# marbl/Mash

Hardware: AMD Instinct MI355X
Metric: pairwise Mash distances/sec (s=1000) (higher is better)
Workload: dtype u64; 1 GPU; mash triangle all-vs-all, 100000 clustered synthetic sketches, k=21 s=1000, 4999950000 pairs/step, per-table job (index build + discover + fill + merge each step), row-block sharded x1; parallelism=rowblock1, rccl_ranks=0

## Files before the change

### mash_amd/csrc/compare_dense.hip

```cpp
#ifdef MG_HIP_EMU
#include "hipemu.h"
#else
#include <hip/hip_runtime.h>
#define MG_DYN_SHARED(T, name)                                   \
    extern __shared__ __align__(16) unsigned char name##_raw[]; \
    T *name = reinterpret_cast<T *>(name##_raw)
#endif
#include <stdint.h>

#include <cstdlib>

#ifndef MG_HIP_EMU
#include <rocprim/device/device_radix_sort.hpp>
#include <rocprim/device/device_select.hpp>
#include <rocprim/iterator/counting_iterator.hpp>
#endif

#include "compare_internal.h"

namespace mg {

#ifndef MG_HIP_EMU
__global__ __launch_bounds__(256) void dn_neighbor_kernel(const uint64_t *hashes, uint64_t stride, const uint32_t *cnt, uint32_t n,
                                                          uint8_t *link)
{
    const uint32_t row = blockIdx.x * 4u + (threadIdx.x >> 6), lane = threadIdx.x & 63u;
    if (row >= n) return;
    uint32_t hit = 0;
    uint32_t ci = 0, cj = 0;
    if (row > 0) {
        ci = cnt[row];
        cj = cnt[row - 1];
        const uint32_t take = ci < 64u ? ci : 64u, span = cj < 256u ? cj : 256u;
        if (lane < take && span > 0) {
            const uint64_t v = hashes[(uint64_t)row * stride + lane];
            const uint64_t *q = hashes + (uint64_t)(row - 1) * stride;
            uint32_t lo = 0, hi = span;
            while (lo < hi) {
                const uint32_t mid = (lo + hi) >> 1;
                if (q[mid] < v) lo = mid + 1; else hi = mid;
            }
            hit = (lo < span && q[lo] == v) ? 1u : 0u;
        }
    }
    const uint32_t hits = (uint32_t)__popcll(__ballot(hit != 0));
    const uint32_t take = ci < 64u ? ci : 64u;
    if (lane == 0) link[row] = (row > 0 && take >= 16u && cj >= 16u && 2u * hits >= take) ? 1 : 0;
}

hipError_t launch_dense_neighbors(const uint64_t *hashes, uint64_t stride, const uint32_t *cnt, uint32_t n, uint8_t *link,
                                  hipStream_t stream)
{
    if (n == 0) return hipSuccess;
    hipLaunchKernelGGL(dn_neighbor_kernel, dim3((n + 3u) / 4u), dim3(256), 0, stream, hashes, stride, cnt, n, link);
    return hipGetLastError();
}

constexpr uint32_t DN_SUBLISTS = 1024;

__global__ __launch_bounds__(256) void dn_leaders_kernel(const uint32_t *sorted_rows, const uint32_t *gs_of, const uint32_t *gend,
                                                         const uint32_t *grp_of, const DenseGroup *groups, uint32_t E,
                                                         unsigned long long *key, uint32_t *val, uint32_t cap_sub, uint32_t *cnt)
{
    const uint32_t pos = blockIdx.x * 256u + threadIdx.x;
    bool lead = false;
    uint32_t g = 0xFFFFFFFFu, gs = 0;
    if (pos < E) {
        g = grp_of[sorted_rows[pos]];
        if (g != 0xFFFFFFFFu) {
            const uint32_t g0 = groups[g].g0, g1 = groups[g].g1;
            gs = gs_of[pos];
            const bool first = pos == gs || sorted_rows[pos - 1] < g0;
            const bool more = pos + 1u < gend[gs] && sorted_rows[pos + 1] < g1;
            lead = first && more;
        }
    }
    const uint64_t bal = __ballot(lead);
    if (bal == 0) return;
    const uint32_t lane = threadIdx.x & 63u, sub = blockIdx.x & (DN_SUBLISTS - 1u);
    uint32_t base = 0;
    if (lane == (uint32_t)__builtin_ctzll(bal)) base = atomicAdd(&cnt[sub], (uint32_t)__popcll(bal));
    base = (uint32_t)__builtin_amdgcn_readlane((int)base, __builtin_ctzll(bal));
    if (lead) {
        const uint32_t k = base + (uint32_t)__popcll(bal & ((1ull << lane) - 1ull));
        if (k < cap_sub) {
            const uint64_t slot = (uint64_t)sub * cap_sub + k;
            key[slot] = ((unsigned long long)g << 32) | gs;
            val[slot] = pos;
        }
    }
}

__global__ __launch_bounds__(DN_SUBLISTS) void dn_sublists_scan_kernel(const uint32_t *cnt, uint32_t cap_sub, uint32_t *off, uint32_t *total)
{
    __shared__ uint32_t s_w[DN_SUBLISTS / 64];
    const uint32_t t = threadIdx.x, lane = t & 63u, wid = t >> 6;
    const uint32_t want = cnt[t], c = want < cap_sub ? want : cap_sub;
    uint32_t incl = c;
#pragma unroll
    for (int d = 1; d < 64; d <<= 1) {
        const uint32_t x = __shfl_up(incl, d);
        if (lane >= (uint32_t)d) incl += x;
    }
    if (lane == 63u) s_w[wid] = incl;
    __syncthreads();
    uint32_t base = 0;
    for (uint32_t k = 0; k < wid; k++) base += s_w[k];
    off[t] = base + incl - c;
    if (t == DN_SUBLISTS - 1u) total[0] = base + incl;
    atomicMax(&total[1], want);
}

__global__ __launch_bounds__(256) void dn_sublists_copy_kernel(const unsigned long long *key, const uint32_t *val, const uint32_t *cnt,
                                                               const uint32_t *off, uint32_t cap_sub, unsigned long long *key_out,
                                                               uint32_t *val_out)
{
    const uint32_t sub = blockIdx.x;
    const uint32_t c = cnt[sub] < cap_sub ? cnt[sub] : cap_sub, o = off[sub];
    for (uint32_t k = threadIdx.x; k < c; k += 256u) {
        key_out[o + k] = key[(uint64_t)sub * cap_sub + k];
        val_out[o + k] = val[(uint64_t)sub * cap_sub + k];
    }
}

__global__ __launch_bounds__(256) void dn_universe_split_kernel(const unsigned long long *key_sorted, uint32_t m, uint32_t *ulist,
                                                                uint32_t *ustart, uint32_t *uend)
{
    const uint32_t i = blockIdx.x * 256u + threadIdx.x;
    if (i >= m) return;
    const unsigned long long k = key_sorted[i];
    const uint32_t g = (uint32_t)(k >> 32);
    ulist[i] = (uint32_t)k;
    if (i == 0 || (uint32_t)(key_sorted[i - 1] >> 32) != g) ustart[g] = i;
    if (i + 1u == m || (uint32_t)(key_sorted[i + 1] >> 32) != g) uend[g] = i + 1u;
}

size_t dense_universe_temp_bytes(uint32_t cap)
{
    size_t b = 0;
    rocprim::radix_sort_pairs(nullptr, b, (const unsigned long long *)nullptr, (unsigned long long *)nullptr, (const uint32_t *)nullptr,
                              (uint32_t *)nullptr, (size_t)cap, 0u, 64u, (hipStream_t) nullptr);
    return b;
}

uint32_t dense_sublists() { return DN_SUBLISTS; }

hipError_t dense_find_leaders(const uint32_t *sorted_rows, const uint32_t *gs_of, const uint32_t *gend, const uint32_t *grp_of,
                              const DenseGroup *groups, uint32_t E, unsigned long long *key, uint32_t *val, uint32_t cap_sub,
                              unsigned long long *key_out, uint32_t *val_out, uint32_t *cnt, uint32_t *off, uint32_t *total,
                              hipStream_t stream)
{
    if (E == 0) return hipSuccess;
    hipError_t e = hipMemsetAsync(cnt, 0, DN_SUBLISTS * 4, stream);
    if (e == hipSuccess) e = hipMemsetAsync(total, 0, 8, stream);
    if (e != hipSuccess) return e;
    hipLaunchKernelGGL(dn_leaders_kernel, dim3((E + 255u) / 256u), dim3(256), 0, stream, sorted_rows, gs_of, gend, grp_of, groups, E, key, val, cap_sub,
                       cnt);
    e = hipGetLastError();
    if (e != hipSuccess) return e;
    return dense_join_leaders(key, val, cap_sub, key_out, val_out, cnt, off, total, stream);
}

hipError_t dense_join_leaders(const unsigned long long *key, const uint32_t *val, uint32_t cap_sub, unsigned long long *key_out, uint32_t *val_out,
                              const uint32_t *cnt, uint32_t *off, uint32_t *total, hipStream_t stream)
{
    hipLaunchKernelGGL(dn_sublists_scan_kernel, dim3(1), dim3(DN_SUBLISTS), 0, stream, cnt, cap_sub, off, total);
    hipLaunchKernelGGL(dn_sublists_copy_kernel, dim3(DN_SUBLISTS), dim3(256), 0, stream, key, val, cnt, (const uint32_t *)off, cap_sub, key_out, val_out);
    return hipGetLastError();
}

hipError_t dense_sort_universes(const unsigned long long *key, const uint32_t *val, uint32_t m, void *temp, size_t temp_bytes,
                                unsigned long long *key_sorted, uint32_t *ulist, uint32_t *upos, uint32_t *ustart, uint32_t *uend,
                                uint32_t group_bits, hipStream_t stream)
{
    if (m == 0) return hipSuccess;
    hipError_t e = rocprim::radix_sort_pairs(temp, temp_bytes, key, key_sorted, val, upos, (size_t)m, 0u, 32u + group_bits, stream);
    if (e != hipSuccess) return e;
    hipLaunchKernelGGL(dn_universe_split_kernel, dim3((m + 255u) / 256u), dim3(256), 0, stream, (const unsigned long long *)key_sorted, m, ulist,
                       ustart, uend);
    return hipGetLastError();
}

#endif

constexpr uint32_t DN_CX_MASK = 0x7FFFu, DN_CX_FLAG = 0x8000u;

struct DnEncodeOpts {
    uint32_t ul_in_lds;
    uint32_t *row_any;
#ifdef __HIPCC__
    __host__ __device__
#endif
    DnEncodeOpts(uint32_t ul, uint32_t *flags = nullptr) : ul_in_lds(ul), row_any(flags) {}
};

template <uint32_t DN_EK>
__global__ __launch_bounds__(256) void dn_encode_kernel(const uint32_t *off, const uint32_t *code_img, uint32_t *pos_img, uint32_t rs,
                                                        const uint32_t *grp_of, const DenseGroup *groups, const uint32_t *ulist,
                                                        const uint32_t *upos, unsigned long long *gdata, uint32_t wstride, uint16_t *ext,
                                                        uint32_t xs, uint32_t n, DnEncodeOpts opt)
{
    MG_DYN_SHARED(uint32_t, lds);
    const uint32_t bid = blockIdx.x;
    const uint32_t row = (bid & ~63u) | ((bid & 7u) << 3) | ((bid >> 3) & 7u);
    const uint32_t tid = threadIdx.x, lane = tid & 63u, wid = tid >> 6;
    if (row >= n) return;
    const uint32_t g = grp_of[row];
    if (g == 0xFFFFFFFFu) return;
    const DenseGroup G = groups[g];
    const uint32_t W = G.W, u = G.u;
    uint32_t *mask32 = lds, *hist = lds + 2u * W, *gap8 = hist + W + 1u, *ovf = gap8 + 16u * W, *pl32 = ovf + W, *scr = pl32 + 8u * W;
    uint32_t *ull = lds + 28u * wstride + 9u;
    for (uint32_t i = tid; i < 28u * W + 1u; i += 256u) lds[i] = 0;
    const uint32_t *ulg = ulist + G.ustart, *up = upos + G.ustart;
    if (opt.ul_in_lds)
        for (uint32_t i = tid; i < u; i += 256u) ull[i] = ulg[i];
    const uint32_t *ul = opt.ul_in_lds ? ull : ulg;
    if (tid == 0) scr[4] = 0;
    __syncthreads();
    const uint32_t cnt = off[row + 1] - off[row];
    uint16_t *xrow = ext + (uint64_t)(G.xrow0 + (row - G.g0)) * xs;
    uint32_t nx = 0;
    bool any = false;
    if constexpr (DN_EK == 1) {
        for (uint32_t base = 0; base < cnt; base += 256u) {
            const uint32_t p = base + tid;
            uint32_t idx = 0;
            bool extra = false;
            if (p < cnt) {
                const uint64_t img = (uint64_t)row * rs + p;
                const uint32_t code = code_img[img], gs = code >> 1;
                uint32_t lo = 0, hi = u;
                while (lo < hi) {
                    const uint32_t mid = (lo + hi) >> 1;
                    if (ul[mid] < gs) lo = mid + 1; else hi = mid;
                }
                idx = lo;
                if (lo < u && ul[lo] == gs) {
                    atomicOr(&mask32[idx >> 5], 1u << (idx & 31u));
                    const uint32_t end = up[idx];
                    pos_img[img] = end;
                    any |= end != gs;
                } else {
                    extra = true;
                    if (opt.row_any && (code & 1u)) any |= pos_img[img] != gs;
                }
            }
            const uint64_t bal = __ballot(extra);
            const uint32_t before = (uint32_t)__popcll(bal & ((1ull << lane) - 1ull));
            if (lane == 0) scr[wid] = (uint32_t)__popcll(bal);
            __syncthreads();
            uint32_t woff = 0;
            for (uint32_t k = 0; k < wid; k++) woff += scr[k];
            const uint32_t total = scr[0] + scr[1] + scr[2] + scr[3];
            if (extra) {
                xrow[nx + woff + before] = (uint16_t)idx;
                atomicAdd(&hist[idx >> 6], 1u);
                atomicAdd(&gap8[idx >> 2], 1u << (8u * (idx & 3u)));
            }
            nx += total;
            __syncthreads();
        }
    } else {
        for (uint32_t base = 0; base < cnt; base += 256u * DN_EK) {
            const uint32_t p0 = base + tid * DN_EK;
            const uint32_t nv = p0 < cnt ? (cnt - p0 < DN_EK ? cnt - p0 : DN_EK) : 0u;
            uint32_t xidx[DN_EK];
            uint32_t nxt = 0;
            if (nv) {
                const uint64_t img0 = (uint64_t)row * rs + p0;
                const uint4 c0 = *reinterpret_cast<const uint4 *>(code_img + img0), c1 = *reinterpret_cast<const uint4 *>(code_img + img0 + 4u);
                const uint32_t code[DN_EK] = {c0.x, c0.y, c0.z, c0.w, c1.x, c1.y, c1.z, c1.w};
                uint4 *pp = reinterpret_cast<uint4 *>(pos_img + img0);
                const uint4 q0 = pp[0], q1 = pp[1];
                uint32_t pv[DN_EK] = {q0.x, q0.y, q0.z, q0.w, q1.x, q1.y, q1.z, q1.w};
                uint32_t pos = 0;
                {
                    const uint32_t gs0 = code[0] >> 1;
                    uint32_t lo = 0, hi = u;
                    while (lo < hi) {
                        const uint32_t mid = (lo + hi) >> 1;
                        if (ul[mid] < gs0) lo = mid + 1; else hi = mid;
                    }
                    pos = lo;
                }
    #pragma unroll
                for (uint32_t e = 0; e < DN_EK; e++) {
                    if (e < nv) {
                        const uint32_t gs = code[e] >> 1;
                        {
                            uint32_t lo = pos, hi = pos, step = 1;
                            while (hi < u && ul[hi] < gs) {
                                lo = hi + 1u;
                                hi += step;
                                step <<= 1;
                            }
                            hi = hi < u ? hi : u;
                            while (lo < hi) {
                                const uint32_t mid = (lo + hi) >> 1;
                                if (ul[mid] < gs) lo = mid + 1u; else hi = mid;
                            }
                            pos = lo;
                        }
                        if (pos < u && ul[pos] == gs) {
                            atomicOr(&mask32[pos >> 5], 1u << (pos & 31u));
                            pv[e] = up[pos];
                        } else {
    #pragma unroll
                            for (uint32_t j = 0; j < DN_EK; j++)
                                if (j == nxt) xidx[j] = pos;
                            nxt++;
                        }
                        any |= pv[e] != gs;
                    }
                }
                pp[0] = make_uint4(pv[0], pv[1], pv[2], pv[3]);
                pp[1] = make_uint4(pv[4], pv[5], pv[6], pv[7]);
            }
            uint32_t incl = nxt;
    #pragma unroll
            for (uint32_t d = 1; d < 64u; d <<= 1) {
                const uint32_t y = __shfl_up(incl, d);
                if (lane >= d) incl += y;
            }
            if (lane == 63u) scr[wid] = incl;
            __syncthreads();
            uint32_t woff = 0;
            for (uint32_t k = 0; k < wid; k++) woff += scr[k];
            const uint32_t total = scr[0] + scr[1] + scr[2] + scr[3];
            const uint32_t at0 = nx + woff + incl - nxt;
    #pragma unroll
            for (uint32_t j = 0; j < DN_EK; j++) {
                if (j < nxt) {
                    const uint32_t idx = xidx[j];
                    xrow[at0 + j] = (uint16_t)idx;
                    atomicAdd(&hist[idx >> 6], 1u);
                    atomicAdd(&gap8[idx >> 2], 1u << (8u * (idx & 3u)));
                }
            }
            nx += total;
            __syncthreads();
        }
    }
    if (__ballot(any) != 0 && lane == 0) atomicOr(&scr[4], 1u);
    __syncthreads();
    if (opt.row_any && tid == 0) opt.row_any[row] = scr[4];
    const uint32_t jb = (row - G.g0) >> 7, bl = (row - G.g0) & 127u;
    const uint64_t bw = dense_block_words(W);
    unsigned long long *blk = gdata + G.data_off + (uint64_t)jb * bw;
    uint16_t *cxp = reinterpret_cast<uint16_t *>(blk + 128ull * W), *totp = cxp + (W + 1u) * 128u;
    unsigned long long *xpl = blk + dense_block_planes(W);
    for (uint32_t i = tid; i < 16u * W; i += 256u) {
        const uint32_t four = gap8[i], w = i >> 4, q = i & 15u;
        uint32_t bits[4] = {0u, 0u, 0u, 0u}, over = 0;
#pragma unroll
        for (uint32_t e = 0; e < 4u; e++) {
            const uint32_t c = (four >> (8u * e)) & 255u;
            over |= c >= 16u ? 1u : 0u;
#pragma unroll
            for (uint32_t j = 0; j < 4u; j++) bits[j] |= ((c >> j) & 1u) << ((4u * q + e) & 31u);
        }
        if (over || (q == 0 && hist[w] >= 256u)) ovf[w] = 1u;
#pragma unroll
        for (uint32_t j = 0; j < 4u; j++)
            if (bits[j]) atomicOr(&pl32[2u * (4u * w + j) + (q >> 3)], bits[j]);
    }
    __syncthreads();
    for (uint32_t i = tid; i < 4u * W; i += 256u) xpl[i * 128u + bl] = (unsigned long long)pl32[2u * i] | ((unsigned long long)pl32[2u * i + 1u] << 32);
    if (tid == 0) {
        uint32_t run = 0, all = 0;
        for (uint32_t w = 0; w <= W; w++) {
            cxp[w * 128u + bl] = (uint16_t)(run | ((w > 0 && ovf[w - 1u]) ? DN_CX_FLAG : 0u));
            totp[w * 128u + bl] = (uint16_t)all;
            if (w < W) {
                run += hist[w];
                all += hist[w] + (uint32_t)__popc(mask32[2u * w]) + (uint32_t)__popc(mask32[2u * w + 1u]);
            }
        }
    }
    for (uint32_t w = tid; w < W; w += 256u)
        blk[w * 128u + bl] = (unsigned long long)mask32[2u * w] | ((unsigned long long)mask32[2u * w + 1u] << 32);
}

hipError_t launch_dense_encode(const uint32_t *off, const uint32_t *code_img, uint32_t *pos_img, uint32_t rs, const uint32_t *grp_of,
                               const DenseGroup *groups, const uint32_t *ulist, const uint32_t *upos, unsigned long long *gdata,
                               uint16_t *ext, uint32_t xs, uint32_t n, uint32_t wmax, hipStream_t stream, int ul_mode, uint32_t *row_any)
{
    if (n == 0) return hipSuccess;
    const size_t fixed = ((size_t)28 * wmax + 9) * 4, with_ul = fixed + (size_t)wmax * 64 * 4;
    const bool ul_in_lds = ul_mode == 0 ? false : ul_mode == 1 ? with_ul <= 150 * 1024 : with_ul <= 40 * 1024;
    const size_t smem = ul_in_lds ? with_ul : fixed;
    auto go = [&](auto kern) -> hipError_t {
        hipError_t e = hipFuncSetAttribute(reinterpret_cast<const void *>(kern), hipFuncAttributeMaxDynamicSharedMemorySize, (int)smem);
        if (e != hipSuccess) return e;
        hipLaunchKernelGGL(kern, dim3((n + 63u) & ~63u), dim3(256), smem, stream, off, code_img, pos_img, rs, grp_of, groups, ulist, upos, gdata, wmax, ext, xs,
                           n, DnEncodeOpts(ul_in_lds ? 1u : 0u, row_any));
        return hipGetLastError();
    };
    return rs >= 4096u ? go(dn_encode_kernel<8>) : go(dn_encode_kernel<1>);
}



__device__ __forceinline__ uint32_t dn_count_add(uint32_t x, uint32_t acc)
{
#ifdef MG_HIP_EMU
    return (uint32_t)__popc(x) + acc;
#else
    uint32_t d;
    asm("v_bcnt_u32_b32 %0, %1, %2" : "=v"(d) : "v"(x), "v"(acc));
    return d;
#endif
}

__device__ __forceinline__ uint32_t dn_low_bits(uint32_t x, uint32_t y)
{
#ifdef MG_HIP_EMU
    return x & ((1u << y) - 1u);
#else
    return __builtin_amdgcn_ubfe(x, 0u, y);
#endif
}

template <uint32_t NP>
__device__ __forceinline__ uint32_t dn_descend(uint32_t base, uint32_t s, uint32_t u1, uint32_t A0, uint32_t B0, uint32_t A1, uint32_t B1,
                                               uint32_t A2, uint32_t B2, uint32_t A3, uint32_t B3)
{
    uint32_t pos = 0;
#pragma unroll
    for (uint32_t bit = 16u; bit != 0u; bit >>= 1) {
        const uint32_t y = pos + bit;
        uint32_t c = dn_count_add(dn_low_bits(B0, y), dn_count_add(dn_low_bits(A0, y), dn_count_add(dn_low_bits(u1, y), base)));
        if (NP >= 1u) c += 2u * dn_count_add(dn_low_bits(B1, y), (uint32_t)__popc(dn_low_bits(A1, y)));
        if (NP >= 3u)
            c += 4u * dn_count_add(dn_low_bits(B2, y), (uint32_t)__popc(dn_low_bits(A2, y))) +
                 8u * dn_count_add(dn_low_bits(B3, y), (uint32_t)__popc(dn_low_bits(A3, y)));
        pos = c < s ? y : pos;
    }
    return pos;
}

__device__ __forceinline__ uint32_t dn_resolve(unsigned long long un, unsigned long long mab, uint32_t fprev, uint32_t s, uint32_t w, bool lists,
                                               const unsigned long long *xpa, const unsigned long long *xpb, const uint16_t *xa,
                                               const uint16_t *xb, uint32_t ca0, uint32_t na, uint32_t cb0, uint32_t nb)
{
    if (__ballot(lists) == 0) {
        const unsigned long long a0 = xpa[512u * w], a1 = xpa[512u * w + 128u], a2 = xpa[512u * w + 256u], a3 = xpa[512u * w + 384u];
        const unsigned long long b0 = xpb[512u * w], b1 = xpb[512u * w + 128u], b2 = xpb[512u * w + 256u], b3 = xpb[512u * w + 384u];
        const bool p1 = __ballot((a1 | b1) != 0ull) != 0, p23 = __ballot((a2 | a3 | b2 | b3) != 0ull) != 0;
        const uint32_t ulo = (uint32_t)un, uhi = (uint32_t)(un >> 32);
        uint32_t c31 = dn_count_add((uint32_t)b0, dn_count_add((uint32_t)a0, dn_count_add(ulo & 0x7FFFFFFFu, fprev)));
        if (p1 || p23) c31 += 2u * dn_count_add((uint32_t)b1, (uint32_t)__popc((uint32_t)a1));
        if (p23)
            c31 += 4u * dn_count_add((uint32_t)b2, (uint32_t)__popc((uint32_t)a2)) + 8u * dn_count_add((uint32_t)b3, (uint32_t)__popc((uint32_t)a3));
        const bool upper = c31 < s;
        const uint32_t base = upper ? c31 + (ulo >> 31) : fprev;
        const uint32_t u1 = (upper ? uhi : ulo) << 1;
        const uint32_t A0 = upper ? (uint32_t)(a0 >> 32) : (uint32_t)a0, B0 = upper ? (uint32_t)(b0 >> 32) : (uint32_t)b0;
        uint32_t pos;
        if (!p1 && !p23) {
            pos = dn_descend<0>(base, s, u1, A0, B0, 0, 0, 0, 0, 0, 0);
        } else {
            const uint32_t A1 = upper ? (uint32_t)(a1 >> 32) : (uint32_t)a1, B1 = upper ? (uint32_t)(b1 >> 32) : (uint32_t)b1;
            if (!p23) {
                pos = dn_descend<1>(base, s, u1, A0, B0, A1, B1, 0, 0, 0, 0);
            } else {
                const uint32_t A2 = upper ? (uint32_t)(a2 >> 32) : (uint32_t)a2, B2 = upper ? (uint32_t)(b2 >> 32) : (uint32_t)b2;
                const uint32_t A3 = upper ? (uint32_t)(a3 >> 32) : (uint32_t)a3, B3 = upper ? (uint32_t)(b3 >> 32) : (uint32_t)b3;
                pos = dn_descend<3>(base, s, u1, A0, B0, A1, B1, A2, B2, A3, B3);
            }
        }
        const uint32_t mlo = (uint32_t)mab, mhi = (uint32_t)(mab >> 32);
        return upper ? dn_count_add(dn_low_bits(mhi, pos), (uint32_t)__popc(mlo)) : (uint32_t)__popc(dn_low_bits(mlo, pos));
    }
    uint32_t lo = 0, hi = 63;
    const uint32_t wbase = w << 6;
    while (lo < hi) {
        const uint32_t mid = (lo + hi) >> 1;
        uint32_t c = fprev + (uint32_t)__popcll(un & ((1ull << mid) - 1ull));
        for (uint32_t k = 0; k < na; k++) c += ((uint32_t)xa[ca0 + k] - wbase <= mid) ? 1u : 0u;
        for (uint32_t k = 0; k < nb; k++) c += ((uint32_t)xb[cb0 + k] - wbase <= mid) ? 1u : 0u;
        if (c >= s) hi = mid; else lo = mid + 1u;
    }
    return (uint32_t)__popcll(mab & ((1ull << lo) - 1ull));
}

template <uint32_t DN_ROWS, uint32_t DN_IL>
__global__ __launch_bounds__(128) void dn_pairs_kernel(const DenseTile *tiles, const DenseGroup *groups, const unsigned long long *gdata,
                                                       uint32_t use_lists,
                                                       const uint16_t *ext, uint32_t xs, uint32_t s, uint32_t row_begin, uint32_t row_end,
                                                       uint64_t out_base, const uint32_t *inv, uint2 *out, DenseList list)
{
    MG_DYN_SHARED(unsigned long long, dl);
    const DenseTile T = tiles[blockIdx.x];
    const DenseGroup G = groups[T.group];
    const uint32_t W = G.W, tid = threadIdx.x;
    const uint64_t bw = dense_block_words(W);
    const unsigned long long *Bm = gdata + G.data_off + (uint64_t)T.cblk * bw;
    const uint16_t *Bcx = reinterpret_cast<const uint16_t *>(Bm + 128ull * W);
    const uint16_t *Btot = Bcx + (W + 1u) * 128u;
    unsigned long long *Am = dl;
    uint16_t *Acx = reinterpret_cast<uint16_t *>(Am + (uint64_t)DN_ROWS * W);
    uint16_t *Atot = Acx + (W + 1u) * DN_ROWS;
    const uint32_t ra = T.row0 - G.g0;
    const unsigned long long *asrc = gdata + G.data_off + (uint64_t)(ra >> 7) * bw;
    const uint32_t la0 = ra & 127u;
    for (uint32_t i = tid; i < W * DN_ROWS; i += 128u) Am[i] = asrc[(i / DN_ROWS) * 128u + la0 + (i % DN_ROWS)];
    {
        const uint16_t *acs = reinterpret_cast<const uint16_t *>(asrc + 128ull * W);
        for (uint32_t i = tid; i < 2u * (W + 1u) * DN_ROWS; i += 128u) Acx[i] = acs[(i / DN_ROWS) * 128u + la0 + (i % DN_ROWS)];
    }
    __syncthreads();
    constexpr uint32_t DN_NB = DN_ROWS / DN_IL;
    uint16_t *Amax = Atot + (W + 1u) * DN_ROWS;
    for (uint32_t i = tid; i < DN_NB * (W + 1u); i += 128u) {
        const uint32_t bt = i / (W + 1u), w = i - bt * (W + 1u);
        uint32_t m = 0;
        for (uint32_t k = 0; k < DN_IL; k++)
            if (T.row0 + bt * DN_IL + k < G.g1) {
                const uint32_t v = Atot[w * DN_ROWS + bt * DN_IL + k];
                m = v > m ? v : m;
            }
        Amax[i] = (uint16_t)m;
    }
    __syncthreads();
    const uint32_t b = G.g0 + T.cblk * 128u + tid;
    const uint32_t lb = b < G.g1 ? tid : G.g1 - 1u - (G.g0 + T.cblk * 128u);
    const uint16_t *xb = ext + (uint64_t)(G.xrow0 + (b < G.g1 ? b - G.g0 : 0u)) * xs;
    const unsigned long long *xpb = Bm + dense_block_planes(W) + lb;
    const uint32_t colrow = inv ? inv[G.g0 + T.cblk * 128u + lb] : G.g0 + T.cblk * 128u + lb;
    const uint64_t tri_col = (colrow ? (uint64_t)colrow * (colrow - 1u) / 2u : 0ull) - out_base;
    for (uint32_t ai = 0; ai < DN_ROWS; ai += DN_IL) {
        if (T.row0 + ai >= G.g1 || T.row0 + ai >= row_end) break;
        const uint16_t *amax = Amax + (ai / DN_IL) * (W + 1u);
        uint32_t common[DN_IL], nle[DN_IL];
#pragma unroll
        for (uint32_t k = 0; k < DN_IL; k++) common[k] = nle[k] = 0;
        unsigned long long mb_next = Bm[lb];
        uint32_t tb_next = Btot[128u + lb];
        uint32_t wi = 0;
        for (; wi < W; wi++) {
            if (__ballot((uint32_t)amax[wi + 1u] + tb_next > s) != 0) break;
            const unsigned long long mb = mb_next;
            if (wi + 1u < W) {
                mb_next = Bm[(wi + 1u) * 128u + lb];
                tb_next = Btot[(wi + 2u) * 128u + lb];
            }
            const uint32_t mlo = (uint32_t)mb, mhi = (uint32_t)(mb >> 32);
#pragma unroll
            for (uint32_t k = 0; k < DN_IL; k++) {
                const unsigned long long am = Am[wi * DN_ROWS + ai + k];
                common[k] = dn_count_add((uint32_t)am & mlo, dn_count_add((uint32_t)(am >> 32) & mhi, common[k]));
            }
        }
        const uint32_t nfast = wi;
        for (; wi < W; wi++) {
            const unsigned long long mb = mb_next;
            const int32_t tbs = (int32_t)tb_next - (int32_t)s;
            if (wi + 1u < W) {
                mb_next = Bm[(wi + 1u) * 128u + lb];
                tb_next = Btot[(wi + 2u) * 128u + lb];
            }
            const uint32_t mlo = (uint32_t)mb, mhi = (uint32_t)(mb >> 32);
            bool any = false;
#pragma unroll
            for (uint32_t k = 0; k < DN_IL; k++) {
                const unsigned long long am = Am[wi * DN_ROWS + ai + k];
                const uint32_t cnew = dn_count_add((uint32_t)am & mlo, dn_count_add((uint32_t)(am >> 32) & mhi, common[k]));
                const bool before = (int32_t)Atot[(wi + 1u) * DN_ROWS + ai + k] + tbs <= (int32_t)cnew;
                common[k] = before ? cnew : common[k];
                nle[k] += before ? 1u : 0u;
                any = any || before;
            }
            if (__ballot(any) == 0) break;
        }
#pragma unroll
        for (uint32_t k = 0; k < DN_IL; k++) {
            const uint32_t a = T.row0 + ai + k;
            const bool present = a < G.g1 && a < row_end && a >= row_begin && G.g0 + T.cblk * 128u < a;
            if (!present) continue;
            const bool valid = b < a;
            uint32_t denom = s;
            const uint32_t w = nfast + nle[k];
            const bool need = valid && w < W;
            if (__ballot(need) != 0) {
                const uint32_t wc = need ? w : 0u;
                const unsigned long long ma = Am[wc * DN_ROWS + ai + k], mb = Bm[wc * 128u + lb];
                const uint32_t ca0 = Acx[wc * DN_ROWS + ai + k] & DN_CX_MASK, ca1r = Acx[(wc + 1u) * DN_ROWS + ai + k];
                const uint32_t cb0 = Bcx[wc * 128u + lb] & DN_CX_MASK, cb1r = Bcx[(wc + 1u) * 128u + lb];
                const uint32_t fprev = (uint32_t)Atot[wc * DN_ROWS + ai + k] + (uint32_t)Btot[wc * 128u + lb] - common[k];
                const bool lists = need && (use_lists || ((ca1r | cb1r) & DN_CX_FLAG) != 0);
                const uint32_t add = dn_resolve(ma | mb, ma & mb, fprev, s, wc, lists, asrc + dense_block_planes(W) + la0 + ai + k, xpb,
                                               ext + (uint64_t)(G.xrow0 + (a - G.g0)) * xs, xb, ca0, need ? (ca1r & DN_CX_MASK) - ca0 : 0u, cb0,
                                               need ? (cb1r & DN_CX_MASK) - cb0 : 0u);
                if (need) common[k] += add;
            }
            if (!valid) continue;
            if (w >= W) {
                const uint32_t total = (uint32_t)Atot[W * DN_ROWS + ai + k] + (uint32_t)Btot[W * 128u + lb] - common[k];
                denom = total < s ? total : s;
            }
            if (list.rc) {
                const uint32_t ra = a - list.row_first;
                const uint32_t at = list.row_base[ra] + list.row_cnt[ra] - (a - b);
                list.rc[at] = make_uint2(a, b);
                list.counts[at] = make_uint2(common[k], denom);
            } else {
                const uint32_t arow = inv ? inv[a] : a;
                const uint64_t tri_a = (uint64_t)arow * (arow - 1u) / 2u - out_base;
                out[arow > colrow ? tri_a + colrow : tri_col + arow] = make_uint2(common[k], denom);
            }
        }
    }
}

uint32_t dense_max_words() { return 400; }

size_t dense_pairs_lds(uint32_t W, uint32_t rows) { return (size_t)rows * W * 8 + (size_t)(W + 1u) * rows * 4 + (size_t)(W + 1u) * 8 * 2 + 16; }

uint32_t dense_rows_per_tile(uint64_t wave_rows) { return wave_rows / 32u >= 16384u ? 32u : 8u; }

hipError_t launch_dense_pairs(const DenseTile *tiles, uint32_t ntiles, uint32_t rows_per_tile, const DenseGroup *groups,
                              const unsigned long long *gdata, bool use_lists, const uint16_t *ext, uint32_t xs,
                              uint32_t s, uint32_t wmax, uint32_t row_begin, uint32_t row_end, uint64_t out_base, const uint32_t *inv, uint2 *out,
                              hipStream_t stream, const DenseList *list)
{
    if (ntiles == 0) return hipSuccess;
    const size_t smem = dense_pairs_lds(wmax, rows_per_tile);
    auto go = [&](auto kern) -> hipError_t {
        hipError_t e = hipFuncSetAttribute(reinterpret_cast<const void *>(kern), hipFuncAttributeMaxDynamicSharedMemorySize, (int)smem);
        if (e != hipSuccess) return e;
        hipLaunchKernelGGL(kern, dim3(ntiles), dim3(128), smem, stream, tiles, groups, gdata, use_lists ? 1u : 0u, ext, xs, s, row_begin, row_end,
                           out_base, inv, out, list ? *list : DenseList());
        return hipGetLastError();
    };
    const uint32_t il = 8;
    if (rows_per_tile == 32u) return il >= 16u ? go(dn_pairs_kernel<32, 16>) : il >= 8u ? go(dn_pairs_kernel<32, 8>) : go(dn_pairs_kernel<32, 4>);
    return il >= 8u ? go(dn_pairs_kernel<8, 8>) : go(dn_pairs_kernel<8, 4>);
}

#ifndef MG_HIP_EMU
constexpr uint32_t CL_FIRST = 4;

__global__ __launch_bounds__(256) void cl_emit_kernel(const uint64_t *hashes, uint64_t stride, const uint32_t *cnt, uint32_t n,
                                                      unsigned long long *key, uint32_t *row_out, uint32_t *label)
{
    const uint32_t i = blockIdx.x * 256u + threadIdx.x;
    if (i >= n * CL_FIRST) return;
    const uint32_t row = i / CL_FIRST, f = i % CL_FIRST;
    key[i] = f < cnt[row] ? (unsigned long long)hashes[(uint64_t)row * stride + f] : ~0ull;
    row_out[i] = row;
    if (f == 0) label[row] = row;
}

__global__ __launch_bounds__(256) void cl_minrow_kernel(const unsigned long long *key_sorted, const uint32_t *row_sorted, uint32_t m,
                                                        uint32_t *label)
{
    const uint32_t i = blockIdx.x * 256u + threadIdx.x;
    if (i >= m) return;
    const unsigned long long k = key_sorted[i];
    if (k == ~0ull) return;
    uint32_t lo = 0, hi = i;
    while (lo < hi) {
        const uint32_t mid = (lo + hi) >> 1;
        if (key_sorted[mid] < k) lo = mid + 1; else hi = mid;
    }
    atomicMin(&label[row_sorted[i]], row_sorted[lo]);
}

__global__ __launch_bounds__(256) void cl_jump_kernel(const uint32_t *in, uint32_t *out, uint32_t n)
{
    const uint32_t i = blockIdx.x * 256u + threadIdx.x;
    if (i < n) out[i] = in[in[i]];
}

__global__ __launch_bounds__(256) void cl_order_keys_kernel(const uint32_t *label, uint32_t n, uint32_t split, unsigned long long *key)
{
    const uint32_t i = blockIdx.x * 256u + threadIdx.x;
    if (i < n) key[i] = ((unsigned long long)(i >= split ? 1u : 0u) << 63) | ((unsigned long long)label[i] << 32) | i;
}

__global__ __launch_bounds__(256) void cl_split_keys_kernel(const unsigned long long *key_sorted, uint32_t n, uint32_t *inv, uint32_t *label_sorted)
{
    const uint32_t i = blockIdx.x * 256u + threadIdx.x;
    if (i < n) {
        inv[i] = (uint32_t)(key_sorted[i] & 0xFFFFFFFFull);
        label_sorted[i] = (uint32_t)(key_sorted[i] >> 32) & 0x7FFFFFFFu;
    }
}

size_t dense_cluster_temp_bytes(uint32_t n)
{
    size_t a = 0, b = 0;
    rocprim::radix_sort_pairs(nullptr, a, (const unsigned long long *)nullptr, (unsigned long long *)nullptr, (const uint32_t *)nullptr,
                              (uint32_t *)nullptr, (size_t)n * CL_FIRST, 0u, 64u, (hipStream_t) nullptr);
    rocprim::radix_sort_keys(nullptr, b, (const unsigned long long *)nullptr, (unsigned long long *)nullptr, (size_t)n, 0u, 64u,
                             (hipStream_t) nullptr);
    return a > b ? a : b;
}

hipError_t dense_cluster_rows(const uint64_t *hashes, uint64_t stride, const uint32_t *cnt, uint32_t n, void *temp, size_t temp_bytes,
                              unsigned long long *key_a, unsigned long long *key_b, uint32_t *row_a, uint32_t *row_b, uint32_t *lab_a,
                              uint32_t *lab_b, uint32_t *inv, uint32_t *label_sorted, hipStream_t stream, uint32_t split)
{
    if (n == 0) return hipSuccess;
    const uint32_t m = n * CL_FIRST;
    hipLaunchKernelGGL(cl_emit_kernel, dim3((m + 255u) / 256u), dim3(256), 0, stream, hashes, stride, cnt, n, key_a, row_a, lab_a);
    hipError_t e = hipGetLastError();
    if (e != hipSuccess) return e;
    e = rocprim::radix_sort_pairs(temp, temp_bytes, (const unsigned long long *)key_a, key_b, (const uint32_t *)row_a, row_b, (size_t)m, 0u, 64u,
                                  stream);
    if (e != hipSuccess) return e;
    hipLaunchKernelGGL(cl_minrow_kernel, dim3((m + 255u) / 256u), dim3(256), 0, stream, (const unsigned long long *)key_b, (const uint32_t *)row_b, m,
                       lab_a);
    hipLaunchKernelGGL(cl_jump_kernel, dim3((n + 255u) / 256u), dim3(256), 0, stream, (const uint32_t *)lab_a, lab_b, n);
    hipLaunchKernelGGL(cl_jump_kernel, dim3((n + 255u) / 256u), dim3(256), 0, stream, (const uint32_t *)lab_b, lab_a, n);
    hipLaunchKernelGGL(cl_order_keys_kernel, dim3((n + 255u) / 256u), dim3(256), 0, stream, (const uint32_t *)lab_a, n, split, key_a);
    e = hipGetLastError();
    if (e != hipSuccess) return e;
    e = rocprim::radix_sort_keys(temp, temp_bytes, (const unsigned long long *)key_a, key_b, (size_t)n, 0u, 64u, stream);
    if (e != hipSuccess) return e;
    hipLaunchKernelGGL(cl_split_keys_kernel, dim3((n + 255u) / 256u), dim3(256), 0, stream, (const unsigned long long *)key_b, n, inv, label_sorted);
    return hipGetLastError();
}

__global__ __launch_bounds__(256) void cl_gather_rows_kernel(const uint64_t *hashes, uint64_t stride, const uint32_t *inv, uint64_t *out)
{
    const uint32_t a = blockIdx.x;
    const uint64_t *src = hashes + (uint64_t)inv[a] * stride;
    uint64_t *dst = out + (uint64_t)a * stride;
    for (uint64_t p = threadIdx.x; p < stride; p += 256u) dst[p] = src[p];
}

hipError_t launch_dense_gather_rows(const uint64_t *hashes, uint64_t stride, const uint32_t *inv, uint32_t n, uint64_t *out, hipStream_t stream)
{
    if (n == 0) return hipSuccess;
    hipLaunchKernelGGL(cl_gather_rows_kernel, dim3(n), dim3(256), 0, stream, hashes, stride, inv, out);
    return hipGetLastError();
}

#endif

__global__ __launch_bounds__(256) void dn_group_rows_kernel(const DenseGroup *groups, uint32_t ng, uint32_t n, uint32_t *grp_of, uint4 *lead_rows)
{
    const uint32_t r = blockIdx.x * 256u + threadIdx.x;
    if (r >= n) return;
    uint32_t lo = 0, hi = ng;
    while (lo < hi) {
        const uint32_t mid = (lo + hi) >> 1;
        if (groups[mid].g0 <= r) lo = mid + 1u;
        else hi = mid;
    }
    uint32_t g = 0xFFFFFFFFu, g0 = 0, g1 = 0;
    if (lo > 0 && r < groups[lo - 1u].g1) {
        g = lo - 1u;
        g0 = groups[g].g0;
        g1 = groups[g].g1;
    }
    grp_of[r] = g;
    lead_rows[r] = make_uint4(g, g0, g1, 0u);
}

hipError_t launch_dense_group_rows(const DenseGroup *groups, uint32_t ng, uint32_t n, uint32_t *grp_of, uint32_t *lead_rows, hipStream_t stream)
{
    if (n == 0) return hipSuccess;
    hipLaunchKernelGGL(dn_group_rows_kernel, dim3((n + 255u) / 256u), dim3(256), 0, stream, groups, ng, n, grp_of, reinterpret_cast<uint4 *>(lead_rows));
    return hipGetLastError();
}

}
```

### mash_amd/csrc/compare_internal.h

```cpp
#pragma once
#ifdef MG_HIP_EMU
#include "hipemu.h"
#else
#include <hip/hip_runtime.h>
#endif
#include <stdint.h>

namespace mg {

struct MergedTile {
    uint32_t rows[32];
    uint32_t col0, col1;
};

struct CompareArgs {
    const uint64_t *row_hashes;
    const uint32_t *row_nhash;
    const uint64_t *col_hashes;
    const uint32_t *col_nhash;
    const uint32_t *row_pfx;
    const uint32_t *col_pfx;
    const MergedTile *mtiles;
    uint2 *out;
    uint64_t row_stride, col_stride;
    uint64_t row_pfx_stride, col_pfx_stride;
    uint64_t row_begin, row_end;
    uint64_t ncols;
    uint64_t out_base;
    uint32_t s;
    uint32_t rows_per_tile;
    uint32_t triangle;
    uint32_t unroll;
    uint32_t pfx_shr;
    uint32_t nbuckets;
    unsigned long long *dbg;
    const uint32_t *row_win;
    const uint32_t *col_win;
    uint32_t win, nwin;
    uint32_t win_lo, win_hi;
    uint32_t win_ecap;
    uint8_t *win_mask;
    uint32_t win_kmax;
    uint32_t xcd_remap;
    uint32_t stage_pack;
};

bool compare_merged_supported(uint32_t s);
uint32_t compare_merged_rows(uint32_t s);
hipError_t launch_compare_merged(const CompareArgs &a, uint32_t ntiles, hipStream_t stream);
uint32_t compare_window_rows(uint32_t s);
uint32_t compare_window_entries();
uint32_t compare_window_row_entries();
hipError_t launch_window_offsets(const uint32_t *pfx, uint64_t pfx_stride, const uint32_t *nhash, uint64_t n, uint32_t s,
                                 uint32_t nwin, uint32_t delta, uint32_t *out, hipStream_t stream);
hipError_t launch_table_max(const uint64_t *hashes, const uint32_t *nhash, uint64_t n, uint64_t stride,
                            unsigned long long *out_max, hipStream_t stream);
hipError_t launch_row_classes(const uint64_t *hashes, const uint32_t *nhash, uint64_t n, uint64_t stride,
                              uint8_t *out, unsigned long long *last_out, hipStream_t stream);
uint64_t compare_pfx_stride(uint64_t s);
hipError_t launch_make_prefix(const uint64_t *hashes, const uint32_t *nhash, uint64_t n, uint64_t s,
                              uint64_t pfx_stride, uint32_t shr, uint32_t *out, hipStream_t stream);
hipError_t launch_compare_generic(const CompareArgs &a, hipStream_t stream);

struct DenseGroup;
struct SparseArgs {
    const uint32_t *sorted_rows;
    const uint32_t *lo_img;
    const uint32_t *hi_img;
    uint32_t lo_shift;
    const uint32_t *row_any = nullptr;
    const uint32_t *off;
    const uint32_t *row_img;
    const uint32_t *col_img;
    const uint32_t *col_cnt_off;
    uint32_t rs_row, rs_col;
    uint32_t row_begin, row_end;
    uint32_t ncols;
    uint32_t triangle;
    uint32_t s;
    uint64_t out_base;
    uint2 *cand;
    uint64_t cand_cap;
    unsigned long long *counters;
    uint2 *out;
    uint2 *res;
    unsigned long long *seg_base;
    uint32_t *seg_cnt;
    uint32_t *chunk_inc;
    const uint32_t *rep;
    const uint32_t *cls_of;
    const uint32_t *cls_off;
    const uint32_t *cls_rows;
    const uint32_t *gend;
    const uint32_t *order;
    const uint32_t *inv;
    const uint32_t *dn_grp_of;
    const DenseGroup *dn_groups;
};
size_t sparse_dup_temp_bytes(uint32_t n);
hipError_t launch_sparse_dup_suspects(const unsigned long long *dig, const uint32_t *cnt, uint32_t n, void *temp, size_t temp_bytes,
                                      unsigned long long *dig_sorted, uint32_t *rows_sorted, uint32_t *flags, uint32_t *nflag,
                                      hipStream_t stream);
size_t sparse_order_temp_bytes(uint32_t n);
hipError_t launch_sparse_row_order(const uint32_t *off, const uint32_t *code_img, const uint32_t *gend, const uint32_t *rep, uint32_t n,
                                   uint32_t rs, void *temp, size_t temp_bytes, unsigned long long *key_a, unsigned long long *key_b,
                                   uint32_t *order, hipStream_t stream);
size_t sparse_order_slice_temp_bytes(uint32_t n);
hipError_t launch_sparse_order_slice(const uint32_t *order, uint32_t n, uint32_t rb, uint32_t re, void *temp, size_t temp_bytes,
                                     uint32_t *out, uint32_t *count_out, hipStream_t stream);
hipError_t launch_sparse_class_pairs(uint2 *out, const uint32_t *cls_rows, const uint32_t *cls_first, const uint32_t *off,
                                     const uint32_t *rep, uint32_t members, uint32_t row_begin, uint32_t row_end, uint64_t out_base,
                                     const uint32_t *inv, hipStream_t stream);
hipError_t launch_sparse_row_digest(const uint64_t *hashes, uint64_t stride, const uint32_t *cnt, uint32_t n,
                                    unsigned long long *digest, hipStream_t stream);
hipError_t launch_sparse_row_gate(const uint64_t *hashes, uint64_t stride, const uint32_t *cnt, uint32_t n, unsigned long long *digest,
                                  hipStream_t stream);
hipError_t launch_sparse_row_equal(const uint64_t *hashes, uint64_t stride, const uint32_t *cnt, const uint2 *pairs, uint32_t npairs,
                                   uint32_t *equal, hipStream_t stream);
hipError_t launch_sparse_row_counts(const uint32_t *nhash, uint32_t n, uint32_t cap, uint32_t *cnt, hipStream_t stream);
size_t sparse_offsets_temp_bytes(uint32_t n);
hipError_t launch_sparse_offsets(const uint32_t *cnt, const uint32_t *inv, uint32_t n, void *temp, uint32_t *off, hipStream_t stream);
size_t sparse_sort_temp_bytes(uint32_t E, uint32_t end_bit, uint32_t begin_bit);
uint32_t sparse_img_stride(uint32_t s);
hipError_t sparse_build_index(const uint64_t *hashes, uint64_t stride, const uint32_t *off, uint32_t n, uint32_t E,
                              uint32_t rs, uint32_t end_bit, void *temp, size_t temp_bytes, uint64_t *keys_a,
                              uint32_t *idx_a, uint64_t *keys_sorted, uint32_t *idx_sorted, uint32_t *head, uint32_t *gs_of,
                              uint32_t *sorted_rows, uint32_t *gend, uint32_t *code_img, uint32_t *pos_img, void *stat_scratch,
                              uint32_t begin_bit, void *tie_scratch, unsigned long long *incidences, uint32_t *max_group, uint32_t *groups,
                              uint32_t *bad, uint32_t *tie_overflow, hipStream_t stream, const uint32_t *rowmap = nullptr);
size_t sparse_stat_scratch_bytes();
uint32_t sparse_sort_begin_bit(uint32_t E, uint32_t end_bit, const char *forced_bits, bool all_bits);
size_t sparse_tie_scratch_bytes();
hipError_t launch_sparse_locate(const uint64_t *qhashes, uint64_t qstride, const uint32_t *qoff, uint32_t q_begin, uint32_t nq,
                                const uint64_t *keys_sorted, const uint32_t *gend, uint32_t E, uint32_t rs, uint32_t *qlo_img,
                                uint32_t *qhi_img, uint32_t *qcode_img, hipStream_t stream);
bool sparse_discover_supported(uint32_t ncols_max);
hipError_t launch_sparse_discover(const SparseArgs &a, bool count_only, hipStream_t stream);
hipError_t launch_sparse_merge(const SparseArgs &a, uint64_t expect, uint32_t cus, hipStream_t stream);
bool sparse_merge_rows_supported(uint32_t rs_row);
size_t sparse_scan_temp_bytes(uint32_t nrows);
hipError_t launch_sparse_merge_rows(const SparseArgs &a, uint64_t expect, uint32_t *chunks, void *temp, size_t temp_bytes,
                                    hipStream_t stream, bool *windowed_out = nullptr);
hipError_t launch_sparse_scatter(const SparseArgs &a, uint64_t expect, uint32_t cus, hipStream_t stream);
size_t sparse_gather_temp_bytes(uint32_t nrows);
hipError_t launch_sparse_gather_rows(const SparseArgs &a, uint32_t *cnt_by_row, uint32_t *row_base, void *temp, size_t temp_bytes, uint32_t row_add,
                                     uint2 *rc_out, uint2 *counts_out, hipStream_t stream);
size_t sparse_edges_temp_bytes(uint64_t K);
uint64_t sparse_edges_blocks(uint64_t K);
hipError_t launch_sparse_list_edges(const uint2 *rc, const uint2 *counts, uint64_t K, uint32_t *blk_cnt, uint32_t *blk_off, void *temp, size_t temp_bytes,
                                    uint4 *edges, unsigned long long *total, hipStream_t stream);
uint64_t sparse_fill_chunks(uint64_t pairs);
constexpr uint32_t kFillStop = 0x80000000u;
hipError_t launch_sparse_fill_chunks(uint2 *out, uint64_t pairs, uint32_t numer, uint32_t denom, uint32_t blocks, uint32_t naps, uint32_t *ctr,
                                     hipStream_t stream, uint32_t threads = 256);
hipError_t launch_sparse_fill_value(uint2 *out, uint64_t pairs, uint32_t numer, uint32_t denom, uint32_t blocks_per_cu, uint32_t cus,
                                    hipStream_t stream);
hipError_t launch_sparse_merge_pack(const SparseArgs &a, uint64_t expect, uint32_t *chunks, void *temp, size_t temp_bytes, bool *used,
                                    hipStream_t stream, uint32_t *pack_min_out = nullptr);
hipError_t launch_sparse_fill_short(uint2 *out, const uint32_t *short_rows, const uint32_t *short_rcnt, uint32_t nshort_rows,
                                    const uint32_t *short_cols, const uint32_t *short_ccnt, uint32_t nshort_cols,
                                    uint32_t row_begin, uint32_t ncols, uint32_t triangle, uint64_t out_base, uint32_t s,
                                    const uint32_t *inv, hipStream_t stream);

struct DenseGroup {
    uint32_t g0, g1;
    uint32_t ustart, u;
    uint32_t W;
    uint32_t xrow0;
    uint64_t data_off;
};
struct DenseTile { uint32_t group, row0, cblk; };
#ifdef __HIPCC__
__host__ __device__
#endif
static inline uint64_t dense_block_planes(uint32_t W) { return 128ull * W + 64ull * (W + 1u); }
#ifdef __HIPCC__
__host__ __device__
#endif
static inline uint64_t dense_block_words(uint32_t W) { return dense_block_planes(W) + 512ull * W; }
struct DenseList {
    const uint32_t *row_base = nullptr, *row_cnt = nullptr;
    uint2 *rc = nullptr, *counts = nullptr;
    uint32_t row_first = 0;
};
hipError_t launch_dense_neighbors(const uint64_t *hashes, uint64_t stride, const uint32_t *cnt, uint32_t n, uint8_t *link,
                                  hipStream_t stream);
size_t dense_universe_temp_bytes(uint32_t cap);
uint32_t dense_sublists();
hipError_t dense_find_leaders(const uint32_t *sorted_rows, const uint32_t *gs_of, const uint32_t *gend, const uint32_t *grp_of,
                              const DenseGroup *groups, uint32_t E, unsigned long long *key, uint32_t *val, uint32_t cap_sub,
                              unsigned long long *key_out, uint32_t *val_out, uint32_t *cnt, uint32_t *off, uint32_t *total,
                              hipStream_t stream);
hipError_t dense_join_leaders(const unsigned long long *key, const uint32_t *val, uint32_t cap_sub, unsigned long long *key_out, uint32_t *val_out,
                              const uint32_t *cnt, uint32_t *off, uint32_t *total, hipStream_t stream);
hipError_t dense_sort_universes(const unsigned long long *key, const uint32_t *val, uint32_t m, void *temp, size_t temp_bytes,
                                unsigned long long *key_sorted, uint32_t *ulist, uint32_t *upos, uint32_t *ustart, uint32_t *uend,
                                uint32_t group_bits, hipStream_t stream);
hipError_t launch_dense_encode(const uint32_t *off, const uint32_t *code_img, uint32_t *pos_img, uint32_t rs, const uint32_t *grp_of,
                               const DenseGroup *groups, const uint32_t *ulist, const uint32_t *upos, unsigned long long *gdata,
                               uint16_t *ext, uint32_t xs, uint32_t n, uint32_t wmax, hipStream_t stream, int ul_mode = -1,
                               uint32_t *row_any = nullptr);
size_t dense_pairs_lds(uint32_t W, uint32_t rows);
uint32_t dense_rows_per_tile(uint64_t wave_rows);
uint32_t dense_max_words();
hipError_t launch_dense_pairs(const DenseTile *tiles, uint32_t ntiles, uint32_t rows_per_tile, const DenseGroup *groups,
                              const unsigned long long *gdata, bool use_lists, const uint16_t *ext, uint32_t xs,
                              uint32_t s, uint32_t wmax, uint32_t row_begin, uint32_t row_end, uint64_t out_base, const uint32_t *inv, uint2 *out,
                              hipStream_t stream, const DenseList *list = nullptr);
size_t dense_cluster_temp_bytes(uint32_t n);
hipError_t dense_cluster_rows(const uint64_t *hashes, uint64_t stride, const uint32_t *cnt, uint32_t n, void *temp, size_t temp_bytes,
                              unsigned long long *key_a, unsigned long long *key_b, uint32_t *row_a, uint32_t *row_b, uint32_t *lab_a,
                              uint32_t *lab_b, uint32_t *inv, uint32_t *label_sorted, hipStream_t stream, uint32_t split = 0);
hipError_t launch_dense_gather_rows(const uint64_t *hashes, uint64_t stride, const uint32_t *inv, uint32_t n, uint64_t *out, hipStream_t stream);
hipError_t launch_dense_group_rows(const DenseGroup *groups, uint32_t ng, uint32_t n, uint32_t *grp_of, uint32_t *lead_rows, hipStream_t stream);

struct JoinSide {
    const uint2 *grp = nullptr;
    const uint32_t *ent = nullptr;
    const uint32_t *goff = nullptr;
    const uint32_t *gend = nullptr;
    const uint32_t *thr = nullptr;
};
struct JoinArgs {
    JoinSide rows, cols;
    const uint32_t *row_cnt_off, *col_cnt_off;
    const uint32_t *rep, *col_rep;
    const uint32_t *inv;
    uint2 *out;
    uint64_t out_base;
    uint64_t ntiles;
    uint32_t ncols;
    uint32_t row_begin, row_end;
    uint32_t bi0;
    uint32_t ncb;
    uint32_t triangle, s;
    uint32_t tiles_per_wg = 1;
};
size_t join_order_temp_bytes(uint32_t nrows);
hipError_t join_order_rows(const uint32_t *img, uint32_t rs, const uint32_t *cnt_off, const uint32_t *rep, const uint32_t *inv, const uint32_t *gend,
                           const uint32_t *sorted_rows, uint32_t nrows, void *temp, size_t temp_bytes, uint32_t *lab, unsigned long long *key_a,
                           unsigned long long *key_b, uint32_t *val_a, uint32_t *perm, uint32_t *src, uint32_t *map, hipStream_t stream, uint32_t split = 0);
uint32_t join_block_rows();
uint32_t join_levels();
size_t join_build_temp_bytes(uint64_t slots);
hipError_t join_build_lists(const uint32_t *img, uint32_t rs, const uint32_t *cnt_off, const uint32_t *rep, uint32_t nrows, uint32_t s, uint32_t E,
                            bool only_shared, void *temp, size_t temp_bytes, unsigned long long *key_a, unsigned long long *key_b, uint32_t *val_a,
                            uint32_t *val_b, uint2 *grp, uint32_t *goff, uint32_t *gend, uint32_t *thr, const uint32_t **ent_out, hipStream_t stream);
hipError_t launch_join_levels(const uint32_t *img, uint32_t rs, const uint32_t *cnt_off, const uint32_t *rep, uint32_t nrows, uint32_t s,
                              uint32_t *thr, hipStream_t stream);
hipError_t launch_join_shared(const uint32_t *lo_img, const uint32_t *hi_img, uint32_t lo_shift, uint32_t rs, const uint32_t *cnt_off,
                              uint32_t row_begin, uint32_t row_end, unsigned long long *sum, hipStream_t stream);
hipError_t launch_join_tiles(const JoinArgs &a, hipStream_t stream);

struct FilterArgs {
    const uint2 *counts;
    const uint32_t *min_numer;
    uint32_t *seg_count;
    unsigned long long *seg_off;
    uint4 *edges;
    uint64_t pairs;
    uint64_t first_row;
    uint64_t ncols;
    uint64_t win_lo, win_n;
    uint32_t s;
    uint32_t triangle;
};
uint64_t filter_segments(uint64_t pairs);
hipError_t launch_filter_count(const FilterArgs &a, unsigned long long *total, hipStream_t stream);
hipError_t launch_filter_write(const FilterArgs &a, hipStream_t stream);

}
```

### mash_amd/csrc/compare_sparse.hip

```cpp
#include <stdint.h>

#include <cstdlib>
#include <cstring>

#include "compare_internal.h"
#ifdef MG_HIP_EMU
#include <numeric>
#define SP_DYN_U32(name, align) MG_DYN_SHARED(uint32_t, name)
#else
#include <hip/hip_runtime.h>
#include <rocprim/device/device_radix_sort.hpp>
#include <rocprim/device/device_scan.hpp>
#include <rocprim/device/device_select.hpp>
#include <rocprim/iterator/counting_iterator.hpp>
#define SP_DYN_U32(name, align) extern __shared__ align uint32_t name[]
#endif
#include "copy_gate.h"

namespace mg {

#ifndef MG_HIP_EMU


__global__ __launch_bounds__(256) void sp_fill_entries_kernel(const uint64_t *hashes, uint64_t stride, const uint32_t *rowmap, const uint32_t *off,
                                                              uint32_t rs, uint64_t *keys, uint32_t *idx)
{
    const uint32_t row = blockIdx.x;
    const uint32_t b = off[row], cnt = off[row + 1] - b;
    const uint64_t *src = hashes + (uint64_t)(rowmap ? rowmap[row] : row) * stride;
    const uint32_t ib = row * rs;
    for (uint32_t p = threadIdx.x; p < cnt; p += 256) {
        keys[b + p] = src[p];
        idx[b + p] = ib + p;
    }
}

__global__ __launch_bounds__(256) void sp_heads_kernel(const uint64_t *keys, const uint32_t *idx, uint32_t E, uint32_t *head,
                                                       uint32_t *bad)
{
    const uint32_t pos = blockIdx.x * 256u + threadIdx.x;
    if (pos >= E) return;
    uint32_t h = pos;
    if (pos > 0) {
        const uint64_t k = keys[pos], kp = keys[pos - 1];
        if (k == kp) {
            h = 0;
            if (idx[pos] <= idx[pos - 1]) *bad = 1;
        } else if (k < kp) {
            *bad = 1;
        }
    }
    head[pos] = h;
}

constexpr uint32_t SP_STAT_SLOTS = 1024;
struct SpStatSlot { unsigned long long inc; uint32_t max_group, groups; };

__global__ __launch_bounds__(256) void sp_index_scatter_kernel(const uint32_t *idx, const uint32_t *gs_of, uint32_t E,
                                                               uint32_t rs, uint32_t *sorted_rows, uint32_t *gend, uint32_t *code_img,
                                                               uint32_t *pos_img, SpStatSlot *stat)
{
    const uint32_t pos = blockIdx.x * 256u + threadIdx.x;
    unsigned long long inc = 0;
    uint32_t glen = 0, heads = 0;
    if (pos < E) {
        const uint32_t i = idx[pos];
        const uint32_t gs = gs_of[pos];
        const bool last = pos + 1u == E || gs_of[pos + 1u] != gs;
        const bool shared = !(last && gs == pos);
        sorted_rows[pos] = i / rs;
        code_img[i] = (gs << 1) | (shared ? 1u : 0u);
        pos_img[i] = pos;
        inc = pos - gs;
        heads = gs == pos ? 1u : 0u;
        if (last) {
            gend[gs] = pos + 1u;
            glen = pos + 1u - gs;
        }
    }
    for (int d = 32; d > 0; d >>= 1) {
        inc += __shfl_xor(inc, d);
        heads += __shfl_xor(heads, d);
        const uint32_t o = __shfl_xor(glen, d);
        glen = o > glen ? o : glen;
    }
    __shared__ unsigned long long s_inc[4];
    __shared__ uint32_t s_len[4], s_heads[4];
    if ((threadIdx.x & 63) == 0) { s_inc[threadIdx.x >> 6] = inc; s_len[threadIdx.x >> 6] = glen; s_heads[threadIdx.x >> 6] = heads; }
    __syncthreads();
    if (threadIdx.x == 0) {
        SpStatSlot *sl = stat + (blockIdx.x & (SP_STAT_SLOTS - 1u));
        const unsigned long long t = s_inc[0] + s_inc[1] + s_inc[2] + s_inc[3];
        uint32_t m = s_len[0];
        for (int w = 1; w < 4; w++) m = s_len[w] > m ? s_len[w] : m;
        if (t) atomicAdd(&sl->inc, t);
        if (m > 1) atomicMax(&sl->max_group, m);
        atomicAdd(&sl->groups, s_heads[0] + s_heads[1] + s_heads[2] + s_heads[3]);
    }
}

__global__ __launch_bounds__(256) void sp_stat_reduce_kernel(const SpStatSlot *stat, unsigned long long *incidences, uint32_t *max_group,
                                                             uint32_t *groups)
{
    unsigned long long inc = 0;
    uint32_t m = 0, g = 0;
    for (uint32_t i = threadIdx.x; i < SP_STAT_SLOTS; i += 256u) {
        inc += stat[i].inc;
        m = stat[i].max_group > m ? stat[i].max_group : m;
        g += stat[i].groups;
    }
    if (inc) atomicAdd(incidences, inc);
    if (m) atomicMax(max_group, m);
    if (g) atomicAdd(groups, g);
}

size_t sparse_stat_scratch_bytes() { return sizeof(SpStatSlot) * SP_STAT_SLOTS; }

__global__ __launch_bounds__(256) void sp_entry_counts_kernel(const uint32_t *nhash, uint32_t n, uint32_t cap, uint32_t *cnt)
{
    const uint32_t i = blockIdx.x * 256u + threadIdx.x;
    if (i < n) cnt[i] = nhash[i] < cap ? nhash[i] : cap;
}

hipError_t launch_sparse_row_counts(const uint32_t *nhash, uint32_t n, uint32_t cap, uint32_t *cnt, hipStream_t stream)
{
    if (n == 0) return hipSuccess;
    hipLaunchKernelGGL(sp_entry_counts_kernel, dim3((n + 255u) / 256u), dim3(256), 0, stream, nhash, n, cap, cnt);
    return hipGetLastError();
}

__global__ __launch_bounds__(1024) void sp_offsets_sums_kernel(const uint32_t *cnt, const uint32_t *inv, uint32_t n, uint32_t *part)
{
    __shared__ uint32_t s_part[16];
    const uint32_t tid = threadIdx.x, a = blockIdx.x * 1024u + tid;
    uint32_t c = a < n ? cnt[inv ? inv[a] : a] : 0u;
#pragma unroll
    for (uint32_t d = 32; d > 0; d >>= 1) c += __shfl_xor(c, d);
    if ((tid & 63u) == 0) s_part[tid >> 6] = c;
    __syncthreads();
    if (tid == 0) {
        uint32_t t = 0;
        for (uint32_t k = 0; k < 16u; k++) t += s_part[k];
        part[blockIdx.x] = t;
    }
}

__global__ __launch_bounds__(1024) void sp_offsets_scan_kernel(const uint32_t *cnt, const uint32_t *inv, uint32_t n, const uint32_t *part, uint32_t *off)
{
    __shared__ uint32_t s_part[16], s_base[16];
    const uint32_t tid = threadIdx.x, lane = tid & 63u, wid = tid >> 6, a = blockIdx.x * 1024u + tid;
    uint32_t before = 0;
    for (uint32_t k = tid; k < blockIdx.x; k += 1024u) before += part[k];
#pragma unroll
    for (uint32_t d = 32; d > 0; d >>= 1) before += __shfl_xor(before, d);
    if (lane == 0) s_base[wid] = before;
    const uint32_t c = a < n ? cnt[inv ? inv[a] : a] : 0u;
    uint32_t incl = c;
#pragma unroll
    for (uint32_t d = 1; d < 64u; d <<= 1) {
        const uint32_t y = __shfl_up(incl, d);
        if (lane >= d) incl += y;
    }
    if (lane == 63u) s_part[wid] = incl;
    __syncthreads();
    uint32_t run = incl - c;
    for (uint32_t k = 0; k < 16u; k++) run += s_base[k] + (k < wid ? s_part[k] : 0u);
    if (a < n) off[a] = run;
    if (a + 1u == n) off[n] = run + c;
}

size_t sparse_offsets_temp_bytes(uint32_t n) { return ((size_t)n / 1024u + 1u) * 4u; }

hipError_t launch_sparse_offsets(const uint32_t *cnt, const uint32_t *inv, uint32_t n, void *temp, uint32_t *off, hipStream_t stream)
{
    if (n == 0) return hipMemsetAsync(off, 0, 4, stream);
    const uint32_t nb = (n + 1023u) / 1024u;
    hipLaunchKernelGGL(sp_offsets_sums_kernel, dim3(nb), dim3(1024), 0, stream, cnt, inv, n, static_cast<uint32_t *>(temp));
    hipLaunchKernelGGL(sp_offsets_scan_kernel, dim3(nb), dim3(1024), 0, stream, cnt, inv, n, static_cast<const uint32_t *>(temp), off);
    return hipGetLastError();
}

#endif

__global__ __launch_bounds__(256) void sp_fill_u32_kernel(uint32_t *p, uint64_t count, uint32_t v)
{
    const uint64_t stride = (uint64_t)gridDim.x * 256u;
    for (uint64_t i = (uint64_t)blockIdx.x * 256u + threadIdx.x; i < count; i += stride) p[i] = v;
}

#ifndef MG_HIP_EMU

__global__ __launch_bounds__(256) void sp_row_digest_kernel(const uint64_t *hashes, uint64_t stride, const uint32_t *cnt,
                                                            unsigned long long *digest)
{
    const uint32_t row = blockIdx.x;
    const uint32_t n = cnt[row];
    const uint64_t *src = hashes + (uint64_t)row * stride;
    unsigned long long h = 0;
    for (uint32_t p = threadIdx.x; p < n; p += 256) {
        unsigned long long z = src[p] + 0x9E3779B97F4A7C15ull * (unsigned long long)(p + 1);
        z = (z ^ (z >> 30)) * 0xBF58476D1CE4E5B9ull;
        z = (z ^ (z >> 27)) * 0x94D049BB133111EBull;
        h += z ^ (z >> 31);
    }
    for (int d = 32; d > 0; d >>= 1) h += __shfl_xor(h, d);
    __shared__ unsigned long long s_h[4];
    if ((threadIdx.x & 63) == 0) s_h[threadIdx.x >> 6] = h;
    __syncthreads();
    if (threadIdx.x == 0) digest[row] = s_h[0] + s_h[1] + s_h[2] + s_h[3];
}

__global__ __launch_bounds__(256) void sp_row_gate_kernel(const uint64_t *hashes, uint64_t stride, const uint32_t *cnt, uint32_t nrows,
                                                          unsigned long long *digest)
{
    static_assert(COPY_GATE_SAMPLES == 32, "half a wave per row");
    const uint32_t row = blockIdx.x * 8u + (threadIdx.x >> 5), k = threadIdx.x & 31u;
    const uint32_t n = row < nrows ? cnt[row] : 0u;
    unsigned long long h = 0;
    if (k < copy_gate_samples(n)) {
        const uint32_t p = copy_gate_position(k, n);
        unsigned long long z = hashes[(uint64_t)row * stride + p] + 0x9E3779B97F4A7C15ull * (unsigned long long)(p + 1);
        z = (z ^ (z >> 30)) * 0xBF58476D1CE4E5B9ull;
        z = (z ^ (z >> 27)) * 0x94D049BB133111EBull;
        h = z ^ (z >> 31);
    }
    for (int d = 16; d > 0; d >>= 1) h += __shfl_xor(h, d);
    if (k == 0 && row < nrows) digest[row] = h;
}

__global__ __launch_bounds__(256) void sp_row_equal_kernel(const uint64_t *hashes, uint64_t stride, const uint32_t *cnt,
                                                           const uint2 *pairs, uint32_t npairs, uint32_t *equal)
{
    const uint32_t k = blockIdx.x;
    if (k >= npairs) return;
    const uint2 pr = pairs[k];
    const uint32_t n = cnt[pr.x];
    int diff = cnt[pr.y] != n;
    const uint64_t *x = hashes + (uint64_t)pr.x * stride, *y = hashes + (uint64_t)pr.y * stride;
    for (uint32_t p = threadIdx.x; p < n && !diff; p += 256) diff |= x[p] != y[p];
    diff = __syncthreads_or(diff);
    if (threadIdx.x == 0) equal[k] = diff ? 0u : 1u;
}

hipError_t launch_sparse_row_digest(const uint64_t *hashes, uint64_t stride, const uint32_t *cnt, uint32_t n,
                                    unsigned long long *digest, hipStream_t stream)
{
    if (n == 0) return hipSuccess;
    hipLaunchKernelGGL(sp_row_digest_kernel, dim3(n), dim3(256), 0, stream, hashes, stride, cnt, digest);
    return hipGetLastError();
}

hipError_t launch_sparse_row_gate(const uint64_t *hashes, uint64_t stride, const uint32_t *cnt, uint32_t n, unsigned long long *digest,
                                  hipStream_t stream)
{
    if (n == 0) return hipSuccess;
    hipLaunchKernelGGL(sp_row_gate_kernel, dim3((n + 7u) / 8u), dim3(256), 0, stream, hashes, stride, cnt, n, digest);
    return hipGetLastError();
}

hipError_t launch_sparse_row_equal(const uint64_t *hashes, uint64_t stride, const uint32_t *cnt, const uint2 *pairs, uint32_t npairs,
                                   uint32_t *equal, hipStream_t stream)
{
    if (npairs == 0) return hipSuccess;
    hipLaunchKernelGGL(sp_row_equal_kernel, dim3(npairs), dim3(256), 0, stream, hashes, stride, cnt, pairs, npairs, equal);
    return hipGetLastError();
}

__global__ __launch_bounds__(256) void sp_dup_flags_kernel(const unsigned long long *dig_sorted, const uint32_t *rows_sorted,
                                                           const uint32_t *cnt, uint32_t n, uint32_t *flags, uint32_t *nflag)
{
    const uint32_t k = blockIdx.x * 256u + threadIdx.x;
    if (k >= n) return;
    uint32_t f = 0;
    if (k > 0 && dig_sorted[k] == dig_sorted[k - 1]) {
        const uint32_t c = cnt[rows_sorted[k]];
        f = (c != 0 && c == cnt[rows_sorted[k - 1]]) ? 1u : 0u;
    }
    flags[k] = f;
    if (f) atomicAdd(nflag, 1u);
}

size_t sparse_dup_temp_bytes(uint32_t n)
{
    size_t b = 0;
    rocprim::radix_sort_pairs(nullptr, b, (const unsigned long long *)nullptr, (unsigned long long *)nullptr,
                              rocprim::counting_iterator<uint32_t>(0u), (uint32_t *)nullptr, (size_t)n, 0u, 64u, (hipStream_t) nullptr);
    return b;
}

hipError_t launch_sparse_dup_suspects(const unsigned long long *dig, const uint32_t *cnt, uint32_t n, void *temp, size_t temp_bytes,
                                      unsigned long long *dig_sorted, uint32_t *rows_sorted, uint32_t *flags, uint32_t *nflag,
                                      hipStream_t stream)
{
    if (n == 0) return hipSuccess;
    hipError_t e = hipMemsetAsync(nflag, 0, 4, stream);
    if (e != hipSuccess) return e;
    e = rocprim::radix_sort_pairs(temp, temp_bytes, dig, dig_sorted, rocprim::counting_iterator<uint32_t>(0u), rows_sorted, (size_t)n, 0u, 64u,
                                  stream);
    if (e != hipSuccess) return e;
    hipLaunchKernelGGL(sp_dup_flags_kernel, dim3((n + 255u) / 256u), dim3(256), 0, stream, dig_sorted, rows_sorted, cnt, n, flags, nflag);
    return hipGetLastError();
}

__global__ __launch_bounds__(256) void sp_row_key_kernel(const uint32_t *off, const uint32_t *code_img, const uint32_t *gend,
                                                         const uint32_t *rep, uint32_t n, uint32_t rs, unsigned long long *key64)
{
    const uint32_t row = blockIdx.x * 4u + (threadIdx.x >> 6), lane = threadIdx.x & 63u;
    if (row >= n) return;
    const uint32_t er = rep ? rep[row] : row;
    const uint32_t cnt = off[er + 1] - off[er];
    uint32_t k = 0xFFFFFFFFu;
    for (uint32_t base = 0; base < cnt; base += 64u) {
        const uint32_t p = base + lane;
        const uint32_t code = p < cnt ? code_img[(uint64_t)er * rs + p] : 0u;
        const uint64_t m = __ballot((code & 1u) != 0);
        if (m != 0) {
            k = (uint32_t)__builtin_amdgcn_readlane((int)code, __builtin_ctzll(m)) >> 1;
            break;
        }
    }
    if (lane == 0) key64[row] = ((unsigned long long)k << 32) | (unsigned long long)(0xFFFFFFFFu - row);
}

__global__ __launch_bounds__(256) void sp_order_from_keys_kernel(const unsigned long long *key64_sorted, uint32_t n, uint32_t *order)
{
    const uint32_t i = blockIdx.x * 256u + threadIdx.x;
    if (i < n) order[i] = 0xFFFFFFFFu - (uint32_t)(key64_sorted[i] & 0xFFFFFFFFull);
}

size_t sparse_order_temp_bytes(uint32_t n)
{
    size_t b = 0;
    rocprim::radix_sort_keys(nullptr, b, (const unsigned long long *)nullptr, (unsigned long long *)nullptr, (size_t)n, 0u, 64u,
                             (hipStream_t) nullptr);
    return b;
}

hipError_t launch_sparse_row_order(const uint32_t *off, const uint32_t *code_img, const uint32_t *gend, const uint32_t *rep, uint32_t n,
                                   uint32_t rs, void *temp, size_t temp_bytes, unsigned long long *key_a, unsigned long long *key_b,
                                   uint32_t *order, hipStream_t stream)
{
    if (n == 0) return hipSuccess;
    hipLaunchKernelGGL(sp_row_key_kernel, dim3((n + 3u) / 4u), dim3(256), 0, stream, off, code_img, gend, rep, n, rs, key_a);
    hipError_t e = hipGetLastError();
    if (e != hipSuccess) return e;
    e = rocprim::radix_sort_keys(temp, temp_bytes, (const unsigned long long *)key_a, key_b, (size_t)n, 0u, 64u, stream);
    if (e != hipSuccess) return e;
    hipLaunchKernelGGL(sp_order_from_keys_kernel, dim3((n + 255u) / 256u), dim3(256), 0, stream, (const unsigned long long *)key_b, n, order);
    return hipGetLastError();
}

struct sp_in_range {
    uint32_t rb, re;
    __device__ bool operator()(const uint32_t &r) const { return r >= rb && r < re; }
};

size_t sparse_order_slice_temp_bytes(uint32_t n)
{
    size_t b = 0;
    rocprim::select(nullptr, b, (const uint32_t *)nullptr, (uint32_t *)nullptr, (uint32_t *)nullptr, (size_t)n, sp_in_range{0u, 0u},
                    (hipStream_t) nullptr);
    return b;
}

hipError_t launch_sparse_order_slice(const uint32_t *order, uint32_t n, uint32_t rb, uint32_t re, void *temp, size_t temp_bytes,
                                     uint32_t *out, uint32_t *count_out, hipStream_t stream)
{
    return rocprim::select(temp, temp_bytes, order, out, count_out, (size_t)n, sp_in_range{rb, re}, stream);
}

#endif

uint32_t sparse_img_stride(uint32_t s) { return ((s + 3u) & ~3u) + 4u; }

#ifndef MG_HIP_EMU
struct sp_max_u32 {
    __device__ uint32_t operator()(const uint32_t &a, const uint32_t &b) const { return a > b ? a : b; }
};

size_t sparse_sort_temp_bytes(uint32_t E, uint32_t end_bit, uint32_t begin_bit)
{
    size_t bytes = 0;
    rocprim::radix_sort_pairs(nullptr, bytes, (const uint64_t *)nullptr, (uint64_t *)nullptr, (const uint32_t *)nullptr,
                              (uint32_t *)nullptr, (size_t)E, 0u, end_bit, (hipStream_t) nullptr);
    size_t b1 = 0;
    rocprim::radix_sort_pairs(nullptr, b1, (const uint64_t *)nullptr, (uint64_t *)nullptr, (const uint32_t *)nullptr,
                              (uint32_t *)nullptr, (size_t)E, begin_bit, end_bit, (hipStream_t) nullptr);
    bytes = bytes > b1 ? bytes : b1;
    size_t b2 = 0;
    rocprim::inclusive_scan(nullptr, b2, (const uint32_t *)nullptr, (uint32_t *)nullptr, (size_t)E, sp_max_u32(), (hipStream_t) nullptr);
    return bytes > b2 ? bytes : b2;
}

constexpr uint32_t SP_TIE_WALK = 1024, SP_TIE_CAP = 1u << 16, SP_TIE_VALUES = 64;

__global__ __launch_bounds__(256) void sp_tie_find_kernel(const uint64_t *keys, uint32_t E, uint32_t bb, uint32_t *breaks, uint32_t *nbreak,
                                                          uint32_t *overflow)
{
    const uint32_t pos = blockIdx.x * 256u + threadIdx.x;
    if (pos == 0 || pos >= E) return;
    const uint64_t k = keys[pos], kp = keys[pos - 1];
    if ((kp >> bb) != (k >> bb) || k == kp) return;
    const uint32_t slot = atomicAdd(nbreak, 1u);
    if (slot >= SP_TIE_CAP) { *overflow = 1; return; }
    breaks[slot] = pos;
}

__global__ __launch_bounds__(64) void sp_tie_segments_kernel(const uint64_t *keys, uint32_t E, uint32_t bb, const uint32_t *breaks,
                                                             const uint32_t *nbreak, uint2 *segs, uint32_t *nseg, uint32_t *overflow)
{
    const uint32_t m = *nbreak < SP_TIE_CAP ? *nbreak : SP_TIE_CAP;
    if (blockIdx.x >= m) return;
    const uint32_t lane = threadIdx.x;
    const uint32_t pos = breaks[blockIdx.x];
    const uint64_t kp = keys[pos - 1];
    const uint64_t prefix = kp >> bb;
    uint32_t s0 = 0;
    {
        uint32_t hi = pos - 1;
        uint32_t chunks = 0;
        for (;;) {
            if (hi == 0) { s0 = 0; break; }
            const bool in = lane < hi;
            const uint64_t k = in ? keys[hi - 1u - lane] : 0;
            const bool other_prefix = in && (k >> bb) != prefix;
            const bool other_value = in && !other_prefix && k != kp;
            const uint64_t stop = __ballot(other_prefix || other_value);
            if (stop) {
                const uint32_t first = (uint32_t)__builtin_ctzll(stop);
                if ((__ballot(other_value) >> first) & 1ull) return;
                s0 = hi - first;
                break;
            }
            if (hi <= 64u) { s0 = 0; break; }
            hi -= 64u;
            if (++chunks > SP_TIE_WALK) { if (lane == 0) *overflow = 1; return; }
        }
    }
    uint32_t s1 = E;
    {
        uint32_t lo = pos;
        uint32_t chunks = 0;
        for (;;) {
            if (lo >= E) { s1 = E; break; }
            const uint32_t q = lo + lane;
            const bool out = q < E && (keys[q] >> bb) != prefix;
            const uint64_t stop = __ballot(out);
            if (stop) { s1 = lo + (uint32_t)__builtin_ctzll(stop); break; }
            lo += 64u;
            if (++chunks > SP_TIE_WALK) { if (lane == 0) *overflow = 1; return; }
        }
    }
    if (lane == 0) segs[atomicAdd(nseg, 1u)] = make_uint2(s0, s1);
}

__global__ __launch_bounds__(64) void sp_tie_repair_kernel(uint64_t *keys, uint32_t *idx, const uint2 *segs, const uint32_t *nseg, uint64_t *tk,
                                                           uint32_t *ti, uint32_t *overflow)
{
    if (blockIdx.x >= *nseg) return;
    const uint32_t lane = threadIdx.x;
    const uint32_t s0 = segs[blockIdx.x].x, s1 = segs[blockIdx.x].y;
    uint32_t out = s0, rounds = 0;
    bool have = false;
    uint64_t last = 0;
    while (out < s1) {
        uint64_t best = ~0ull;
        for (uint32_t q = s0 + lane; q < s1; q += 64u) {
            const uint64_t k = keys[q];
            if ((!have || k > last) && k < best) best = k;
        }
        for (uint32_t d = 32; d; d >>= 1) {
            const uint64_t o = __shfl_xor(best, d, 64);
            best = o < best ? o : best;
        }
        if (++rounds > SP_TIE_VALUES) { if (lane == 0) *overflow = 1; return; }
        for (uint32_t base = s0; base < s1; base += 64u) {
            const uint32_t q = base + lane;
            const bool hit = q < s1 && keys[q] == best;
            const uint64_t bal = __ballot(hit);
            if (hit) {
                const uint32_t w = out + (uint32_t)__popcll(bal & ((1ull << lane) - 1ull));
                tk[w] = best;
                ti[w] = idx[q];
            }
            out += (uint32_t)__popcll(bal);
        }
        last = best;
        have = true;
    }
    __threadfence();
// ... 1106 lines not shown
```

### mash_amd/csrc/host_index.cpp

```cpp
#include "host_internal.h"
#include "index_build.h"
#ifdef IX_PHASE_CLOCKS
namespace mg { void index_dump_clocks(); }
#endif
#include "sort_bits.h"

namespace {

const uint64_t kTilesLongestRun = 6144;
static const uint64_t kSplitMinRun = 128;

uint64_t longest_label_run(const uint32_t *lab_sorted, uint64_t n)
{
    if (!lab_sorted || n == 0) return 0;
    uint64_t run = 1, longest = 1;
    for (uint64_t a = 1; a < n; a++) {
        run = lab_sorted[a] == lab_sorted[a - 1] ? run + 1 : 1;
        longest = std::max(longest, run);
    }
    return longest;
}

struct Carve {
    unsigned char *base = nullptr;
    size_t at = 0;
    template <class T> T *take(size_t count)
    {
        const size_t from = (at + alignof(T) - 1) & ~(alignof(T) - 1);
        at = from + count * sizeof(T);
        return base ? reinterpret_cast<T *>(base + from) : nullptr;
    }
};

struct LeaderLists {
    DevBuf<unsigned long long> key, keyj;
    DevBuf<uint32_t> val, valj, cnt_sub, off_sub, nlead;
    uint32_t lists = mg::dense_sublists(), cap = 0, tot[2] = {0, 0};
    explicit LeaderLists(mg_ctx *c) : key(c), keyj(c), val(c), valj(c), cnt_sub(c), off_sub(c), nlead(c) {}

    hipError_t alloc(uint32_t room)
    {
        key.free(); val.free(); keyj.free(); valj.free();
        const uint64_t all = (uint64_t)lists * room;
        if (!(nlead.p && cnt_sub.p && off_sub.p) && (nlead.alloc(2) != hipSuccess || cnt_sub.alloc(lists) != hipSuccess || off_sub.alloc(lists) != hipSuccess))
            return hipErrorOutOfMemory;
        if (key.alloc(all) != hipSuccess || val.alloc(all) != hipSuccess || keyj.alloc(all) != hipSuccess || valj.alloc(all) != hipSuccess) return hipErrorOutOfMemory;
        cap = room;
        return hipSuccess;
    }
    hipError_t reset(hipStream_t st) { const hipError_t e = hipMemsetAsync(cnt_sub, 0, lists * 4, st); return e != hipSuccess ? e : hipMemsetAsync(nlead, 0, 8, st); }
    hipError_t join(hipStream_t st)
    {
        const hipError_t e = mg::dense_join_leaders(key, val, cap, keyj, valj, cnt_sub, off_sub, nlead, st);
        return e != hipSuccess ? e : hipMemcpyAsync(tot, nlead, 8, hipMemcpyDeviceToHost, st);
    }
    mg::IxLeaders view(const uint32_t *lead_rows) const { return mg::IxLeaders{lead_rows, key, val, cnt_sub, cap, lists}; }
    bool overflowed() const { return tot[1] > cap; }
};

struct SparseIndexBuild {
    mg_ctx *ctx;
    const mg_table *t;
    const uint32_t s;
    const bool clustered;
    const uint32_t split;
    mg_table::Sparse *sp;
    const uint64_t n;
    const std::chrono::steady_clock::time_point t_begin = std::chrono::steady_clock::now();
    bool stop = false;

    bool need_classes = false, dedup = true, want_dense = true, try_cluster = false, try_links = false;
    DevBuf<uint8_t> dc_cls, d_link;
    DevBuf<unsigned long long> dc_last, d_dig, d_dig_sorted, k_a, k_b;
    DevBuf<uint32_t> d_cnt, d_rows_sorted, d_flags, d_nflag, r_a, r_b, l_a, l_b, d_inv, d_lab;
    DevBuf<unsigned char> d_tmp_dup, d_tmp_cl;
    std::vector<uint8_t> hc_cls, link;
    std::vector<uint64_t> hc_last;
    std::vector<uint32_t> hc_nh, inv_v, lab_v;
    const uint32_t *inv = nullptr, *lab_sorted = nullptr;
    uint32_t nflag = 0, gate_suspects = 0;
    size_t tb_dup = 0, tb_cl = 0;
    bool cluster_q = false, links_q = false;

    const char *ix_mode = nullptr;
    bool ix_verify = false, ix_tiles = true;
    std::vector<uint32_t> cnt_true, cnt_perm;
    uint32_t max_cnt = 0;
    uint64_t maxv = 0, E_all = 0;
    double dens[65] = {0};
    double dens0 = 0;
    std::vector<uint32_t> rep;
    const uint64_t *H = nullptr;
    const uint32_t *rowmap = nullptr;
    uint64_t label_run = 0;
    mg::IxPlan early_plan;
    DevBuf<unsigned char> d_lb;
    bool lb_made = false;
    DevBuf<unsigned char> d_tcnt;
    bool cnt_made = false;
    bool cnt_stale = false;

    std::vector<uint32_t> cls_of, cls_off, cls_rows, cls_first;

    uint32_t E = 0, end_bit = 0, sort_begin_bit = 0;
    std::vector<mg::DenseGroup> cand_groups;
    std::vector<uint32_t> grp_of_h;
    DevBuf<mg::DenseGroup> d_groups;
    DevBuf<uint32_t> d_grp_of, d_lead_rows;
    LeaderLists lead;
    bool lead_ready = false, cand_prepared = false;
    mg::IxPlan plan;
    size_t temp_bytes = 0;
    DevBuf<unsigned char> temp;
    DevBuf<uint32_t> gs_of;
    DevBuf<unsigned long long> key64_a, key64_b;
    struct Stat { unsigned long long shared; uint32_t max_group, groups, bad, tie_overflow; uint32_t ixf[4]; } h_stat = {0, 0, 0, 0, 0, {0, 0, 0, 0}};
    DevBuf<Stat> d_stat;
    DevBuf<unsigned char> d_slots;
    bool want_order = true;
    std::vector<uint32_t> short_cnt;

    bool built = false;
    uint64_t dn_xrows = 0, dn_words = 0;

    SparseIndexBuild(mg_ctx *c, const mg_table *tab, uint32_t sketch_size, bool clustered_variant, mg_table::Sparse *index, uint32_t split_row)
        : ctx(c), t(tab), s(sketch_size), clustered(clustered_variant), split(split_row), sp(index), n(tab->n), dc_cls(c), d_link(c), dc_last(c), d_dig(c), d_dig_sorted(c),
          k_a(c), k_b(c), d_cnt(c), d_rows_sorted(c), d_flags(c), d_nflag(c), r_a(c), r_b(c), l_a(c), l_b(c), d_inv(c), d_lab(c), d_tmp_dup(c), d_tmp_cl(c), d_lb(c), d_tcnt(c),
          d_groups(c), d_grp_of(c), d_lead_rows(c), lead(c), temp(c), gs_of(c), key64_a(c), key64_b(c), d_stat(c), d_slots(c)
    {}

    int unusable(const char *why) { sp->usable = false; sp->why = why; stop = true; return MG_OK; }


    bool counts_with_offsets()
    {
        const char *o = ctx_opt(ctx, "MASHGPU_IX_COUNTS");
        if ((o && strcmp(o, "tiles") == 0) || !mg::index_offsets_counts_fits(early_plan.g)) return false;
        if (d_tcnt.alloc(early_plan.cnt_bytes) != hipSuccess || d_stat.alloc(1) != hipSuccess ||
            hipMemsetAsync(d_stat, 0, sizeof(Stat), ctx->stream) != hipSuccess) {
            (void)hipGetLastError();
            d_tcnt.free();
            return false;
        }
        return cnt_made = true;
    }

    hipError_t counts_to_device()
    {
            if (!cnt_stale) return hipSuccess;
            cnt_stale = false;
            return hipMemcpyAsync(d_cnt, cnt_true.data(), n * 4, hipMemcpyHostToDevice, ctx->stream);
    }

    template <class T> bool take(T **p, size_t count)
    {
        void *q = nullptr;
        if (ctx_malloc(ctx, &q, std::max<size_t>(count, 1) * sizeof(T)) != hipSuccess) return false;
        *p = static_cast<T *>(q);
        return true;
    }

    void drop()
    {
            for (void **q : {(void **)&sp->off, (void **)&sp->keys_sorted, (void **)&sp->gend, (void **)&sp->sorted_rows, (void **)&sp->code_img,
                             (void **)&sp->pos_img, (void **)&sp->row_any, (void **)&sp->short_rows, (void **)&sp->short_cnt, (void **)&sp->counters, (void **)&sp->order,
                             (void **)&sp->rep, (void **)&sp->cls_of, (void **)&sp->cls_off, (void **)&sp->cls_rows, (void **)&sp->cls_first})
                if (*q) { ctx_free(ctx, *q); *q = nullptr; }
    }

    int no_memory() { (void)hipGetLastError(); drop(); return unusable("no device memory for the index"); }
    int lost(hipError_t e) { drop(); return fail(ctx, MG_ERR_HIP, std::string("compare (index build): ") + hipGetErrorString(e)); }

    void drop_dense()
    {
        for (void **q : {(void **)&sp->dgroups, (void **)&sp->grp_of, (void **)&sp->gdata, (void **)&sp->ext, (void **)&sp->ulist, (void **)&sp->upos})
            if (*q) { ctx_free(ctx, *q); *q = nullptr; }
        sp->dgroups_host.clear();
    }

    struct TileScratch {
        DevBuf<unsigned char> start, big, pk, tc;
        explicit TileScratch(mg_ctx *c) : start(c), big(c), pk(c), tc(c) {}
    };

    int partition_body()
    {
        const char *o = ctx_opt(ctx, "MASHGPU_IX_PARTITION");
        return o && strcmp(o, "lsd") == 0 ? mg::IX_PART_LSD : mg::IX_PART_RANK;
    }

    hipError_t tiles(const TileScratch &w, int stages)
    {
        const mg::IxLeaders lv = lead.view(d_lead_rows);
        return mg::index_build_mapped(plan, H, rowmap, sp->off, d_lb, d_tcnt, w.start, w.big, w.pk, w.tc, sp->keys_sorted, sp->sorted_rows, sp->gend, gs_of, sp->code_img,
                               sp->pos_img, d_slots, &d_stat.p->shared, &d_stat.p->max_group, &d_stat.p->groups, d_stat.p->ixf, lead_ready ? &lv : nullptr,
                               ctx->stream, stages, sp->row_any, partition_body());
    }
    hipError_t sort_buckets(const TileScratch &w)
    {
        hipError_t e = tiles(w, 2);
        if (e == hipSuccess && lead_ready) e = lead.join(ctx->stream);
        return e != hipSuccess ? e : hipMemcpyAsync(&h_stat, d_stat, sizeof(Stat), hipMemcpyDeviceToHost, ctx->stream);
    }
    hipError_t row_order()
    {
        return mg::launch_sparse_row_order(sp->off, sp->code_img, sp->gend, sp->rep, (uint32_t)n, sp->rs, temp, temp_bytes, key64_a, key64_b, sp->order, ctx->stream);
    }

    int scan_rows();
    int copy_rows();
    int order_rows();
    int find_copies();
    int lay_out();
    void prepare_candidates();
    hipError_t tile_passes();
    int build_by_tiles();
    int build_by_sort();
    int check_build();
    bool search_leaders();
    bool sort_universes(std::vector<uint32_t> &us, std::vector<uint32_t> &ue);
    bool choose_groups(const std::vector<uint32_t> &us, const std::vector<uint32_t> &ue);
    int encode_groups();
    int dense_groups();
    int check_row_flags();
    int run();
};

int SparseIndexBuild::scan_rows()
{
    need_classes = t->cls.size() != n;
    dedup = !ctx_opt(ctx, "MASHGPU_SPARSE_NO_DEDUP");
    want_dense = true;
    if (const char *v = ctx_opt(ctx, "MASHGPU_COMPARE_DENSE")) want_dense = atoi(v) != 0;
    try_cluster = clustered && n >= 16;
    try_links = !try_cluster && want_dense && n >= 8 && s <= 16384;
    tb_dup = mg::sparse_dup_temp_bytes((uint32_t)n);
    tb_cl = mg::dense_cluster_temp_bytes((uint32_t)n);
    if (d_cnt.alloc(n) != hipSuccess || (need_classes && (dc_cls.alloc(n) != hipSuccess || dc_last.alloc(n) != hipSuccess)) ||
        (dedup && (d_dig.alloc(n) != hipSuccess || d_dig_sorted.alloc(n) != hipSuccess || d_rows_sorted.alloc(n) != hipSuccess ||
                   d_flags.alloc(n) != hipSuccess || d_nflag.alloc(1) != hipSuccess || d_tmp_dup.alloc(std::max<size_t>(tb_dup, 16)) != hipSuccess))) {
        (void)hipGetLastError();
        return unusable("no device memory for the index");
    }
    {
        hipError_t e = hipSuccess;
        if (need_classes) {
            hc_cls.resize(n);
            hc_last.resize(n);
            hc_nh.resize(n);
            e = mg::launch_row_classes(t->hashes, t->nhash, n, t->s, dc_cls, dc_last, ctx->stream);
        }
        if (e == hipSuccess) e = mg::launch_sparse_row_counts(t->nhash, (uint32_t)n, (uint32_t)std::min<uint64_t>(t->s, s), d_cnt, ctx->stream);
        if (e == hipSuccess && dedup) {
            e = mg::launch_sparse_row_gate(t->hashes, t->s, d_cnt, (uint32_t)n, d_dig, ctx->stream);
            if (e == hipSuccess)
                e = mg::launch_sparse_dup_suspects(d_dig, d_cnt, (uint32_t)n, d_tmp_dup, tb_dup, d_dig_sorted, d_rows_sorted, d_flags, d_nflag, ctx->stream);
        }
        if (e == hipSuccess && try_cluster) {
            if (k_a.alloc(4 * n) == hipSuccess && k_b.alloc(4 * n) == hipSuccess && r_a.alloc(4 * n) == hipSuccess && r_b.alloc(4 * n) == hipSuccess &&
                l_a.alloc(n) == hipSuccess && l_b.alloc(n) == hipSuccess && d_inv.alloc(n) == hipSuccess && d_lab.alloc(n) == hipSuccess &&
                d_tmp_cl.alloc(std::max<size_t>(tb_cl, 16)) == hipSuccess) {
                e = mg::dense_cluster_rows(t->hashes, t->s, d_cnt, (uint32_t)n, d_tmp_cl, tb_cl, k_a, k_b, r_a, r_b, l_a, l_b, d_inv, d_lab, ctx->stream, split);
                cluster_q = true;
            } else {
                (void)hipGetLastError();
            }
        }
        if (e == hipSuccess && try_links) {
            if (d_link.alloc(n) == hipSuccess) {
                link.resize(n);
                e = mg::launch_dense_neighbors(t->hashes, t->s, d_cnt, (uint32_t)n, d_link, ctx->stream);
                links_q = true;
            } else {
                (void)hipGetLastError();
            }
        }
        unsigned long long *p_last = nullptr;
        uint32_t *p_nh = nullptr, *p_inv = nullptr, *p_lab = nullptr, *p_nflag = nullptr;
        uint8_t *p_cls = nullptr, *p_link = nullptr;
        auto carve = [&](unsigned char *block) {
            Carve c{block};
            p_last = c.take<unsigned long long>(n); p_nh = c.take<uint32_t>(n); p_inv = c.take<uint32_t>(n); p_lab = c.take<uint32_t>(n);
            p_nflag = c.take<uint32_t>(2); p_cls = c.take<uint8_t>(n); p_link = c.take<uint8_t>(n);
            return c.at + 64;
        };
        unsigned char *pin = static_cast<unsigned char *>(ctx_pinned(ctx, carve(nullptr)));
        if (pin) {
            carve(pin);
        } else {
            p_nflag = &nflag;
            if (cluster_q) { inv_v.resize(n); lab_v.resize(n); p_inv = inv_v.data(); p_lab = lab_v.data(); }
            p_nh = hc_nh.data(); p_cls = hc_cls.data(); p_last = reinterpret_cast<unsigned long long *>(hc_last.data()); p_link = link.data();
        }
        if (e == hipSuccess && need_classes) {
            e = hipMemcpyAsync(p_nh, t->nhash, n * 4, hipMemcpyDeviceToHost, ctx->stream);
            if (e == hipSuccess) e = hipMemcpyAsync(p_cls, dc_cls, n, hipMemcpyDeviceToHost, ctx->stream);
            if (e == hipSuccess) e = hipMemcpyAsync(p_last, dc_last, n * 8, hipMemcpyDeviceToHost, ctx->stream);
        }
        if (e == hipSuccess && dedup) e = hipMemcpyAsync(p_nflag, d_nflag, 4, hipMemcpyDeviceToHost, ctx->stream);
        if (e == hipSuccess && cluster_q) {
            e = hipMemcpyAsync(p_inv, d_inv, n * 4, hipMemcpyDeviceToHost, ctx->stream);
            if (e == hipSuccess) e = hipMemcpyAsync(p_lab, d_lab, n * 4, hipMemcpyDeviceToHost, ctx->stream);
        }
        if (e == hipSuccess && links_q) e = hipMemcpyAsync(p_link, d_link, n, hipMemcpyDeviceToHost, ctx->stream);
        const hipError_t es = hipStreamSynchronize(ctx->stream);
        if (e == hipSuccess) e = es;
        if (e == hipSuccess && pin) {
            if (need_classes) {
                memcpy(hc_nh.data(), p_nh, n * 4);
                memcpy(hc_cls.data(), p_cls, n);
                memcpy(hc_last.data(), p_last, n * 8);
            }
            if (dedup) nflag = *p_nflag;
            if (links_q) memcpy(link.data(), p_link, n);
        }
        if (cluster_q) { inv = p_inv; lab_sorted = p_lab; }
        if (e != hipSuccess) return fail(ctx, MG_ERR_HIP, std::string("compare (index: rows, copies, order): ") + hipGetErrorString(e));
    }
    gate_suspects = nflag;
    if (need_classes) {
        t->cls.swap(hc_cls);
        t->last.swap(hc_last);
        t->nh.swap(hc_nh);
    }
    if (!links_q) link.clear();
    return MG_OK;
}

int SparseIndexBuild::order_rows()
{
    ix_mode = ctx_opt(ctx, "MASHGPU_SPARSE_INDEX");
    ix_verify = ix_mode && strcmp(ix_mode, "verify") == 0;
    ix_tiles = !ix_mode || strcmp(ix_mode, "sort") != 0;
    cnt_true.assign(n, 0);
    for (uint64_t i = 0; i < n; i++) {
        const uint32_t c = (uint32_t)std::min<uint64_t>(std::min<uint64_t>(t->nh[i], t->s), s);
        cnt_true[i] = c;
        E_all += c;
        max_cnt = std::max(max_cnt, c);
        if (c) {
            const uint64_t last = t->last[i];
            if (last == MG_HASH_PAD) return unusable("a hash equals the padding value");
            maxv = std::max(maxv, last);
            const double d = (double)c / ((double)last + 1.0);
            dens[64 - __builtin_clzll(last | 1ull)] += d;
            dens0 += d;
        }
    }
    H = t->hashes;
    bool keep_table_order = false;
    const uint64_t run = cluster_q ? longest_label_run(lab_sorted, n) : 0;
    if (cluster_q && split != 0 && lab_sorted && !ctx_opt(ctx, "MASHGPU_SPLIT_ALWAYS") && run * (uint64_t)s < kSplitMinRun * 1000ull) {
        keep_table_order = true;
        lab_sorted = nullptr;
    }
    if (cluster_q) {
        bool identity = true;
        for (uint64_t a = 0; a < n && identity; a++) identity = inv[a] == a;
        if (!identity && !keep_table_order) {
            const char *fc = ctx_opt(ctx, "MASHGPU_COMPARE_ROWCOPY");
            const bool copy_now = fc && atoi(fc) != 0;
            void *pi = nullptr, *ph = nullptr;
            if (ctx_malloc(ctx, &pi, n * 4) != hipSuccess || (copy_now && ctx_malloc(ctx, &ph, std::max<uint64_t>(n * t->s, 1) * 8) != hipSuccess)) {
                (void)hipGetLastError();
                ctx_free(ctx, pi);
                lab_sorted = nullptr;
            } else {
                sp->inv = static_cast<uint32_t *>(pi);
                sp->phashes = static_cast<uint64_t *>(ph);
                HIP_TRY(ctx, hipMemcpyAsync(sp->inv, d_inv, n * 4, hipMemcpyDeviceToDevice, ctx->stream));
                if (ix_tiles && !(dedup && nflag) && E_all > 0 && E_all < (1ull << 31) && run <= kTilesLongestRun) {
                    early_plan = mg::index_plan((uint32_t)n, (uint32_t)E_all, s, sp->rs, t->s, maxv, dens0, ix_verify);
                    if (early_plan.ok && d_lb.alloc(early_plan.lb_bytes) == hipSuccess) {
                        if (copy_now) HIP_TRY(ctx, mg::index_gather_rows(early_plan, t->hashes, sp->inv, d_cnt, sp->phashes, d_lb, ctx->stream));
                        else if (counts_with_offsets()) HIP_TRY(ctx, mg::index_offsets_counts(early_plan, t->hashes, sp->inv, d_cnt, d_lb, d_tcnt, d_stat.p->ixf, ctx->stream));
                        else HIP_TRY(ctx, mg::index_window_offsets(early_plan, t->hashes, sp->inv, d_cnt, d_lb, ctx->stream));
                        lb_made = true;
                    } else {
                        (void)hipGetLastError();
                    }
                }
                if (copy_now) {
                    if (!lb_made) HIP_TRY(ctx, mg::launch_dense_gather_rows(t->hashes, t->s, sp->inv, (uint32_t)n, sp->phashes, ctx->stream));
                    H = sp->phashes;
                } else {
                    rowmap = sp->inv;
                }
                cnt_perm.resize(n);
                for (uint64_t a = 0; a < n; a++) cnt_perm[a] = cnt_true[inv[a]];
                cnt_true.swap(cnt_perm);
                cnt_stale = true;
            }
        }
    } else {
        lab_sorted = nullptr;
    }
    label_run = lab_sorted ? run : 0;
    if (want_dense && n >= 8 && s <= 16384 && lab_sorted) {
        link.assign(n, 0);
        for (uint64_t a = 1; a < n; a++) link[a] = (a != split && lab_sorted[a] == lab_sorted[a - 1] && cnt_true[a] && cnt_true[a - 1]) ? 1 : 0;
    } else if (cluster_q && want_dense && n >= 8 && s <= 16384 && d_link.alloc(n) == hipSuccess) {
        const int rc = copy_rows();
        if (rc != MG_OK || stop) return rc;
        link.resize(n);
        HIP_TRY(ctx, counts_to_device());
        HIP_TRY(ctx, mg::launch_dense_neighbors(H, t->s, d_cnt, (uint32_t)n, d_link, ctx->stream));
        HIP_TRY(ctx, hipMemcpyAsync(link.data(), d_link, n, hipMemcpyDeviceToHost, ctx->stream));
        HIP_TRY(ctx, hipStreamSynchronize(ctx->stream));
    } else if (!links_q) {
        (void)hipGetLastError();
        link.clear();
    }
    return MG_OK;
}

int SparseIndexBuild::copy_rows()
{
    if (!rowmap) return MG_OK;
    void *ph = nullptr;
    if (ctx_malloc(ctx, &ph, std::max<uint64_t>(n * t->s, 1) * 8) != hipSuccess) return no_memory();
    sp->phashes = static_cast<uint64_t *>(ph);
    HIP_TRY(ctx, mg::launch_dense_gather_rows(t->hashes, t->s, rowmap, (uint32_t)n, sp->phashes, ctx->stream));
    H = sp->phashes;
    rowmap = nullptr;
    return MG_OK;
}

int SparseIndexBuild::find_copies()
{
    if (dedup && nflag) {
        const int rc = copy_rows();
        if (rc != MG_OK || stop) return rc;
        HIP_TRY(ctx, counts_to_device());
        HIP_TRY(ctx, mg::launch_sparse_row_digest(H, t->s, d_cnt, (uint32_t)n, d_dig, ctx->stream));
        HIP_TRY(ctx, mg::launch_sparse_dup_suspects(d_dig, d_cnt, (uint32_t)n, d_tmp_dup, tb_dup, d_dig_sorted, d_rows_sorted, d_flags, d_nflag, ctx->stream));
        HIP_TRY(ctx, hipMemcpyAsync(&nflag, d_nflag, 4, hipMemcpyDeviceToHost, ctx->stream));
        HIP_TRY(ctx, hipStreamSynchronize(ctx->stream));
        if (nflag) {
            std::vector<uint32_t> rows_sorted(n), flags(n);
            HIP_TRY(ctx, hipMemcpyAsync(rows_sorted.data(), d_rows_sorted, n * 4, hipMemcpyDeviceToHost, ctx->stream));
            HIP_TRY(ctx, hipMemcpyAsync(flags.data(), d_flags, n * 4, hipMemcpyDeviceToHost, ctx->stream));
            HIP_TRY(ctx, hipStreamSynchronize(ctx->stream));
            std::vector<uint2> pairs;
            pairs.reserve(nflag);
            for (uint64_t k = 1, g0 = 0; k < n; k++) {
                if (flags[k]) pairs.push_back(make_uint2(rows_sorted[k], rows_sorted[g0]));
                else g0 = k;
            }
            DevBuf<uint2> d_pairs(ctx);
            DevBuf<uint32_t> d_eq(ctx);
            if (d_pairs.alloc(pairs.size()) != hipSuccess || d_eq.alloc(pairs.size()) != hipSuccess) { (void)hipGetLastError(); return unusable("no device memory for the index"); }
            std::vector<uint32_t> eq(pairs.size());
            HIP_TRY(ctx, hipMemcpyAsync(d_pairs, pairs.data(), pairs.size() * sizeof(uint2), hipMemcpyHostToDevice, ctx->stream));
            HIP_TRY(ctx, mg::launch_sparse_row_equal(H, t->s, d_cnt, d_pairs, (uint32_t)pairs.size(), d_eq, ctx->stream));
            HIP_TRY(ctx, hipMemcpyAsync(eq.data(), d_eq, pairs.size() * 4, hipMemcpyDeviceToHost, ctx->stream));
            HIP_TRY(ctx, hipStreamSynchronize(ctx->stream));
            for (size_t k = 0; k < pairs.size(); k++)
                if (eq[k]) {
                    if (rep.empty()) { rep.resize(n); for (uint64_t i = 0; i < n; i++) rep[i] = (uint32_t)i; }
                    rep[pairs[k].x] = pairs[k].y;
                    sp->copies++;
                }
        }
    }
    if (sp->copies) {
        cls_of.assign(n, 0xFFFFFFFFu);
        std::vector<uint32_t> size(n, 0);
        for (uint64_t i = 0; i < n; i++) size[rep[i]]++;
        uint32_t ncls = 0, tot = 0;
        for (uint64_t i = 0; i < n; i++)
            if (size[i] >= 2) { cls_of[i] = ncls++; cls_off.push_back(tot); tot += size[i]; }
        cls_off.push_back(tot);
        cls_rows.resize(tot);
        std::vector<uint32_t> fillp(cls_off.begin(), cls_off.end() - 1);
        for (uint64_t i = 0; i < n; i++) {
            const uint32_t k = cls_of[rep[i]];
            if (k != 0xFFFFFFFFu) cls_rows[fillp[k]++] = (uint32_t)i;
        }
        cls_first.resize(tot);
        for (uint32_t k = 0; k < ncls; k++) {
            const uint64_t m = cls_off[k + 1] - cls_off[k];
            sp->cls_pairs += m * (m - 1) / 2;
            for (uint32_t u = cls_off[k]; u < cls_off[k + 1]; u++) cls_first[u] = cls_off[k];
        }
        sp->cls_members = tot;
        if (ncls == 1 && tot == n && cnt_true[0] > 0) sp->one_class = (uint32_t)cnt_true[0];
        if (sp->one_class && ctx->aside_all_copies) ctx->aside_all_copies(sp->one_class);
    }
    return MG_OK;
}

int SparseIndexBuild::lay_out()
{
    uint64_t E64 = 0;
    sp->off_host.resize(n + 1);
    for (uint64_t i = 0; i < n; i++) {
        sp->off_host[i] = (uint32_t)E64;
        const uint64_t c = cnt_true[i];
        if (rep.empty() || rep[i] == i) E64 += c;
        if (E64 >= (1ull << 31)) return unusable("2^31 entries or more");
        if (c < s) sp->short_rows_host.push_back((uint32_t)i);
        if (c == 0) sp->has_empty = true;
    }
    sp->off_host[n] = (uint32_t)E64;
    if (E64 == 0) return unusable("no hashes");
    E = (uint32_t)E64;
    sp->E = E;
    end_bit = (uint32_t)(64 - __builtin_clzll(maxv | 1ull));
    sort_begin_bit = mg::sparse_sort_begin_bit(E, end_bit, ctx_opt(ctx, "MASHGPU_SPARSE_SORT_BITS"), ctx_opt(ctx, "MASHGPU_SPARSE_SORT_ALL_BITS") != nullptr);
    if (sort_begin_bit > 0 && !ctx_opt(ctx, "MASHGPU_SPARSE_SORT_BITS")) sort_begin_bit = mg::sort_begin_bit_from_density(dens, end_bit, sort_begin_bit);
    const bool tiles_hopeless = ix_tiles && !ix_verify && lab_sorted && !ctx_opt(ctx, "MASHGPU_SPARSE_INDEX") &&
                                label_run > kTilesLongestRun;
    if (ix_tiles && !tiles_hopeless) plan = mg::index_plan((uint32_t)n, E, s, sp->rs, t->s, maxv, dens0, ix_verify);
    else if (tiles_hopeless) plan.why = "a clade of more rows than a bucket's sort takes";
    if (lb_made && !(plan.ok && memcmp(&plan.g, &early_plan.g, sizeof plan.g) == 0)) lb_made = cnt_made = false;
    temp_bytes = std::max(std::max(mg::sparse_order_temp_bytes((uint32_t)n), mg::sparse_order_slice_temp_bytes((uint32_t)n)),
                          mg::sparse_offsets_temp_bytes((uint32_t)n));
    want_order = !ctx_opt(ctx, "MASHGPU_SPARSE_NO_ORDER");
    bool ok = temp.alloc(std::max<size_t>(temp_bytes, 16)) == hipSuccess && gs_of.alloc(E) == hipSuccess && (d_stat.p || d_stat.alloc(1) == hipSuccess) &&
              d_slots.alloc(std::max(mg::sparse_stat_scratch_bytes(), mg::index_stat_scratch_bytes())) == hipSuccess &&
              (!want_order || (key64_a.alloc(n) == hipSuccess && key64_b.alloc(n) == hipSuccess));
    ok = ok && take(&sp->off, n + 1) && take(&sp->keys_sorted, E) && take(&sp->gend, E) && take(&sp->sorted_rows, E) &&
         take(&sp->code_img, (size_t)n * sp->rs + 64) && take(&sp->pos_img, (size_t)n * sp->rs) && take(&sp->row_any, n) && take(&sp->counters, 4) &&
         (!want_order || take(&sp->order, n));
    const size_t nshort = sp->short_rows_host.size();
    short_cnt.assign(nshort, 0);
    for (size_t k = 0; k < nshort; k++) short_cnt[k] = cnt_true[sp->short_rows_host[k]];
    if (ok && nshort) ok = take(&sp->short_rows, nshort) && take(&sp->short_cnt, nshort);
    if (ok && sp->copies)
        ok = take(&sp->rep, n) && take(&sp->cls_of, n) && take(&sp->cls_off, cls_off.size()) && take(&sp->cls_rows, cls_rows.size()) &&
             take(&sp->cls_first, cls_first.size());
    if (!ok) return no_memory();
    hipError_t e = hipSuccess;
    auto upload = [&](uint32_t *dst, const std::vector<uint32_t> &v) {
        if (e == hipSuccess && !v.empty()) e = hipMemcpyAsync(dst, v.data(), v.size() * 4, hipMemcpyHostToDevice, ctx->stream);
    };
    if (sp->copies) { upload(sp->rep, rep); upload(sp->cls_of, cls_of); upload(sp->cls_off, cls_off); upload(sp->cls_rows, cls_rows); upload(sp->cls_first, cls_first); }
    if (!rep.empty()) upload(sp->off, sp->off_host);
    else if (e == hipSuccess) e = mg::launch_sparse_offsets(d_cnt, cnt_stale ? sp->inv : nullptr, (uint32_t)n, temp, sp->off, ctx->stream);
    upload(sp->short_rows, sp->short_rows_host); upload(sp->short_cnt, short_cnt);
    return e == hipSuccess ? MG_OK : lost(e);
}

void SparseIndexBuild::prepare_candidates()
{
    if (cand_prepared) return;
    cand_prepared = true;
    if (link.empty() || sp->copies != 0) return;
    for (uint64_t i = 1; i < n;) {
        if (!link[i]) { i++; continue; }
        uint64_t j = i;
        while (j < n && link[j]) j++;
        if (j - (i - 1) >= 8) {
            mg::DenseGroup g{};
            g.g0 = (uint32_t)(i - 1); g.g1 = (uint32_t)j;
            cand_groups.push_back(g);
        }
        i = j + 1;
    }
    if (cand_groups.empty()) return;
    const uint32_t ng = (uint32_t)cand_groups.size();
    grp_of_h.assign(n, 0xFFFFFFFFu);
    for (uint32_t g = 0; g < ng; g++)
        for (uint32_t r = cand_groups[g].g0; r < cand_groups[g].g1; r++) grp_of_h[r] = g;
    uint32_t room = std::max<uint32_t>(E / 4u / lead.lists + 64u, 256u);
    if (const char *ev = ctx_opt(ctx, "MASHGPU_DENSE_LEAD_CAP")) room = std::max<uint32_t>((uint32_t)atoi(ev), 1u);
    if (d_groups.alloc(ng) == hipSuccess && d_grp_of.alloc(n) == hipSuccess && d_lead_rows.alloc(4 * n) == hipSuccess && lead.alloc(room) == hipSuccess &&
        hipMemcpyAsync(d_groups, cand_groups.data(), ng * sizeof(mg::DenseGroup), hipMemcpyHostToDevice, ctx->stream) == hipSuccess &&
        mg::launch_dense_group_rows(d_groups, ng, (uint32_t)n, d_grp_of, d_lead_rows, ctx->stream) == hipSuccess && lead.reset(ctx->stream) == hipSuccess) {
        lead_ready = true;
    } else {
        (void)hipGetLastError();
        cand_groups.clear();
    }
}

hipError_t SparseIndexBuild::tile_passes()
{
    TileScratch w(ctx);
    if (!((lb_made || d_lb.alloc(plan.lb_bytes) == hipSuccess) && (cnt_made || d_tcnt.alloc(plan.cnt_bytes) == hipSuccess) && w.start.alloc(plan.start_bytes) == hipSuccess &&
          w.big.alloc(plan.big_bytes) == hipSuccess && w.pk.alloc(plan.pk_bytes) == hipSuccess && w.tc.alloc(plan.tc_bytes) == hipSuccess)) {
        (void)hipGetLastError();
        return hipSuccess;
    }
    hipError_t e = cnt_made ? hipSuccess : hipMemsetAsync(d_stat, 0, sizeof(Stat), ctx->stream);
    if (e == hipSuccess) e = tiles(w, cnt_made ? 1 | 8 | 16 : lb_made ? 1 | 8 : 1);
    DevBuf<uint32_t> d_swapped(ctx);
    if (e == hipSuccess && ctx_opt(ctx, "MASHGPU_IX_DEBUG_SWAP") && d_swapped.alloc(1) == hipSuccess) {
        e = hipMemsetAsync(d_swapped, 0, 4, ctx->stream);
        if (e == hipSuccess) e = mg::index_debug_swap(plan, w.pk, w.start, d_swapped, ctx->stream);
    }
    if (e == hipSuccess) prepare_candidates();
    if (e == hipSuccess && ctx->aside_at_sort) ctx->aside_at_sort();
    if (e == hipSuccess) e = sort_buckets(w);
    hipEvent_t ev_stats = nullptr;
    if (e == hipSuccess) e = hipEventCreateWithFlags(&ev_stats, hipEventDisableTiming);
    if (e == hipSuccess) e = hipEventRecord(ev_stats, ctx->stream);
    if (e == hipSuccess) e = tiles(w, 4);
    if (e == hipSuccess && want_order) e = row_order();
    const hipError_t ew = e == hipSuccess ? hipEventSynchronize(ev_stats) : hipStreamSynchronize(ctx->stream);
    if (e == hipSuccess) e = ew;
    if (ev_stats) (void)hipEventDestroy(ev_stats);
    built = e == hipSuccess && !h_stat.ixf[mg::IXF_DEGENERATE];
    if (built && lead_ready && lead.overflowed() && h_stat.ixf[mg::IXF_NBIG] == 0) {
        e = hipStreamSynchronize(ctx->stream);
        const uint32_t want_cap = lead.tot[1];
        if (e == hipSuccess && lead.alloc(want_cap) == hipSuccess) {
            e = lead.reset(ctx->stream);
            if (e == hipSuccess) e = hipMemsetAsync(d_stat.p, 0, offsetof(Stat, bad), ctx->stream);
            if (e == hipSuccess) e = sort_buckets(w);
            if (e == hipSuccess) e = hipStreamSynchronize(ctx->stream);
            built = e == hipSuccess && !h_stat.ixf[mg::IXF_DEGENERATE];
            if (ctx_opt(ctx, "MASHGPU_SPARSE_DBG"))
                fprintf(stderr, "compare dense: a list of leaders asked for %u entries: found again with that room (%u leaders)\n", want_cap, lead.tot[0]);
        } else {
            (void)hipGetLastError();
        }
    }
    if (ctx_opt(ctx, "MASHGPU_SPARSE_DBG"))
        fprintf(stderr, "compare sparse: index by tiles: shift %u, %u buckets (%u per window, %u windows), fullest %u, %u beyond the LDS (%u values streamed)%s\n",
                plan.g.shift, plan.g.Bp, plan.g.BW, plan.g.NW, h_stat.ixf[mg::IXF_MAXBUCKET], h_stat.ixf[mg::IXF_NBIG], h_stat.ixf[mg::IXF_NSTREAMED],
                h_stat.ixf[mg::IXF_DEGENERATE] ? " -- clumped values: sorted instead" : "");
    if (ctx_opt(ctx, "MASHGPU_SPARSE_DBG"))
        fprintf(stderr, "compare sparse: block counts %s\n", cnt_made ? "made with the window offsets (one read of the table)" : "by the tiles (K1)");
    if (ctx_opt(ctx, "MASHGPU_SPARSE_DBG"))
        fprintf(stderr, "compare sparse: tile partition %s\n", partition_body() == mg::IX_PART_LSD ? "by the LSD sort in LDS (lsd)" : "by ranks in registers (rank)");
    return e;
}

int SparseIndexBuild::build_by_tiles()
{
    hipError_t e = hipSuccess;
    if (plan.ok) e = tile_passes();
    else if (ix_tiles && ctx_opt(ctx, "MASHGPU_SPARSE_DBG")) fprintf(stderr, "compare sparse: index by tiles refused: %s\n", plan.why);
    if (e != hipSuccess) return lost(e);
    sp->by_tiles = built;
    prepare_candidates();
#ifdef IX_PHASE_CLOCKS
    if (built && ctx_opt(ctx, "MASHGPU_IX_CLOCKS")) mg::index_dump_clocks();
#endif
    if (ix_verify && !built && !ctx_opt(ctx, "MASHGPU_SPARSE_INDEX_MAY_REFUSE"))
        return fail(ctx, MG_ERR_INVALID, std::string("index verify: the tile build refused this table (") + (plan.ok ? "bucket flags" : plan.why) + ")");
    return MG_OK;
}

int SparseIndexBuild::build_by_sort()
{
    if (built && !ix_verify) return MG_OK;
    const size_t sort_bytes = mg::sparse_sort_temp_bytes(E, end_bit, sort_begin_bit);
    DevBuf<unsigned char> temp_sort(ctx), d_ties(ctx);
    DevBuf<uint64_t> keys_a(ctx), v_keys(ctx);
    DevBuf<uint32_t> idx_a(ctx), idx_sorted(ctx), v_rows(ctx), v_gend(ctx), v_gs(ctx), v_code(ctx), v_pos(ctx);
    DevBuf<unsigned long long> d_diff(ctx);
    bool ok = temp_sort.alloc(std::max<size_t>(sort_bytes, 16)) == hipSuccess && keys_a.alloc(E) == hipSuccess && idx_a.alloc(E) == hipSuccess &&
              idx_sorted.alloc(E) == hipSuccess && d_ties.alloc(mg::sparse_tie_scratch_bytes()) == hipSuccess;
    if (ok && built)
        ok = v_keys.alloc(E) == hipSuccess && v_rows.alloc(E) == hipSuccess && v_gend.alloc(E) == hipSuccess && v_gs.alloc(E) == hipSuccess &&
             v_code.alloc((size_t)n * sp->rs + 64) == hipSuccess && v_pos.alloc((size_t)n * sp->rs) == hipSuccess && d_diff.alloc(16) == hipSuccess;
    if (!ok) return no_memory();
    const Stat tiles_stat = h_stat;
    uint64_t *o_keys = built ? v_keys.p : sp->keys_sorted;
    uint32_t *o_rows = built ? v_rows.p : sp->sorted_rows, *o_gend = built ? v_gend.p : sp->gend, *o_gs = built ? v_gs.p : gs_of.p,
             *o_code = built ? v_code.p : sp->code_img, *o_pos = built ? v_pos.p : sp->pos_img;
    hipError_t e = hipSuccess;
    for (uint32_t begin_bit = sort_begin_bit;; begin_bit = 0) {
        e = hipMemsetAsync(d_stat, 0, sizeof(Stat), ctx->stream);
        if (e == hipSuccess)
            e = mg::sparse_build_index(H, t->s, sp->off, (uint32_t)n, E, sp->rs, end_bit, temp_sort, sort_bytes, keys_a, idx_a, o_keys, idx_sorted,
                                       idx_a, o_gs, o_rows, o_gend, o_code, o_pos, d_slots, begin_bit, d_ties, &d_stat.p->shared,
                                       &d_stat.p->max_group, &d_stat.p->groups, &d_stat.p->bad, &d_stat.p->tie_overflow, ctx->stream, rowmap);
        if (e == hipSuccess && !built && want_order) e = row_order();
        if (e == hipSuccess) e = hipMemcpyAsync(&h_stat, d_stat, sizeof(Stat), hipMemcpyDeviceToHost, ctx->stream);
        if (e == hipSuccess) e = hipStreamSynchronize(ctx->stream);
        if (e != hipSuccess) return lost(e);
        if ((!h_stat.tie_overflow && !h_stat.bad) || begin_bit == 0) break;
        if (ctx_opt(ctx, "MASHGPU_SPARSE_DBG"))
            fprintf(stderr, "compare sparse: sort on bits [%u, %u) %s: every bit again\n", begin_bit, end_bit,
                    h_stat.bad ? "left values out of order" : "left ties the repair could not take");
    }
    if (!built) return MG_OK;
    unsigned long long diff[16];
    for (int k = 0; k < 8; k++) { diff[2 * k] = 0; diff[2 * k + 1] = ~0ull; }
    e = hipMemcpyAsync(d_diff, diff, sizeof diff, hipMemcpyHostToDevice, ctx->stream);
    const uint64_t img = (uint64_t)n * sp->rs;
    const struct { const char *name; const uint32_t *tiles, *sort, *ref; uint32_t mode; uint64_t words; } arrays[6] = {
        {"values (32-bit words)", (const uint32_t *)sp->keys_sorted, (const uint32_t *)v_keys.p, nullptr, 0, 2ull * E}, {"rows", sp->sorted_rows, v_rows, nullptr, 0, E},
        {"group starts", gs_of, v_gs, nullptr, 0, E}, {"group ends", sp->gend, v_gend, v_gs, 1, E}, {"code image", sp->code_img, v_code, nullptr, 0, img},
        {"position image", sp->pos_img, v_pos, v_code, 2, img}};
    for (int k = 0; k < 6 && e == hipSuccess; k++)
        e = mg::index_verify_words(arrays[k].tiles, arrays[k].sort, arrays[k].ref, arrays[k].mode, arrays[k].words, d_diff.p + 2 * k, ctx->stream);
    if (e == hipSuccess) e = hipMemcpyAsync(diff, d_diff, sizeof diff, hipMemcpyDeviceToHost, ctx->stream);
    if (e == hipSuccess) e = hipStreamSynchronize(ctx->stream);
    if (e != hipSuccess) return lost(e);
    std::string msg;
    for (int k = 0; k < 6; k++)
        if (diff[2 * k]) msg += std::string(msg.empty() ? "" : "; ") + arrays[k].name + ": " + std::to_string(diff[2 * k]) + " differ, first at " + std::to_string(diff[2 * k + 1]);
    if (h_stat.shared != tiles_stat.shared || h_stat.max_group != tiles_stat.max_group || h_stat.groups != tiles_stat.groups)
        msg += std::string(msg.empty() ? "" : "; ") + "statistics: shared " + std::to_string(tiles_stat.shared) + " / " + std::to_string(h_stat.shared) +
               ", largest group " + std::to_string(tiles_stat.max_group) + " / " + std::to_string(h_stat.max_group) + ", groups " +
               std::to_string(tiles_stat.groups) + " / " + std::to_string(h_stat.groups);
    if (!msg.empty()) {
        char geom[160];
        snprintf(geom, sizeof geom, " [n %llu, E %u, shift %u, %u buckets, %u per window, %u windows]", (unsigned long long)n, E, plan.g.shift, plan.g.Bp, plan.g.BW, plan.g.NW);
        sp->usable = false;
        return fail(ctx, MG_ERR_INVALID, "index verify: tiles / sort -- " + msg + geom);
    }
    return MG_OK;
}

int SparseIndexBuild::check_build()
{
    if (h_stat.bad) { drop(); return unusable("sort order inside a value not by row"); }
    sp->G = h_stat.groups;
    sp->shared = h_stat.shared;
    sp->max_group = h_stat.max_group;
    sp->build_ms = std::chrono::duration<double, std::milli>(std::chrono::steady_clock::now() - t_begin).count();
    sp->usable = true;
    return MG_OK;
}

bool SparseIndexBuild::search_leaders()
{
    for (int attempt = 0;; attempt++) {
        hipError_t e = mg::dense_find_leaders(sp->sorted_rows, gs_of, sp->gend, d_grp_of, d_groups, E, lead.key, lead.val, lead.cap, lead.keyj, lead.valj,
                                              lead.cnt_sub, lead.off_sub, lead.nlead, ctx->stream);
        if (e == hipSuccess) e = hipMemcpyAsync(lead.tot, lead.nlead, 8, hipMemcpyDeviceToHost, ctx->stream);
        if (e == hipSuccess) e = hipStreamSynchronize(ctx->stream);
        if (e != hipSuccess) return false;
        if (!lead.overflowed() || attempt >= 1) return true;
        if (lead.alloc(lead.tot[1]) != hipSuccess) return false;
    }
}

bool SparseIndexBuild::sort_universes(std::vector<uint32_t> &us, std::vector<uint32_t> &ue)
{
    const uint32_t ng = (uint32_t)cand_groups.size(), nlead = lead.tot[0];
    uint32_t gbits = 1;
    while ((1u << gbits) < ng) gbits++;
    const size_t tb = mg::dense_universe_temp_bytes(nlead);
    DevBuf<uint32_t> d_us(ctx), d_ue(ctx);
    DevBuf<unsigned long long> d_key2(ctx);
    DevBuf<unsigned char> d_utmp(ctx);
    bool ok = d_us.alloc(ng) == hipSuccess && d_ue.alloc(ng) == hipSuccess && d_key2.alloc(nlead) == hipSuccess && d_utmp.alloc(std::max<size_t>(tb, 16)) == hipSuccess;
    if (!ok || !take(&sp->ulist, nlead) || !take(&sp->upos, nlead)) return false;
    hipError_t e = hipMemsetAsync(d_us, 0, ng * 4, ctx->stream);
    if (e == hipSuccess) e = hipMemsetAsync(d_ue, 0, ng * 4, ctx->stream);
    if (e == hipSuccess) e = mg::dense_sort_universes(lead.keyj, lead.valj, nlead, d_utmp, tb, d_key2, sp->ulist, sp->upos, d_us, d_ue, gbits, ctx->stream);
    if (e == hipSuccess) e = hipMemcpyAsync(us.data(), d_us, ng * 4, hipMemcpyDeviceToHost, ctx->stream);
    if (e == hipSuccess) e = hipMemcpyAsync(ue.data(), d_ue, ng * 4, hipMemcpyDeviceToHost, ctx->stream);
    if (e == hipSuccess) e = hipStreamSynchronize(ctx->stream);
    return e == hipSuccess;
}

bool SparseIndexBuild::choose_groups(const std::vector<uint32_t> &us, const std::vector<uint32_t> &ue)
{
    const uint32_t kMaxWords = mg::dense_max_words();
    std::fill(grp_of_h.begin(), grp_of_h.end(), 0xFFFFFFFFu);
    for (uint32_t g = 0; g < (uint32_t)cand_groups.size(); g++) {
        mg::DenseGroup G = cand_groups[g];
        G.u = ue[g] > us[g] ? ue[g] - us[g] : 0u;
        G.ustart = us[g];
        G.W = (G.u >> 6) + 1u;
        if (G.u < 32u || G.W > kMaxWords) continue;
        G.xrow0 = (uint32_t)dn_xrows;
        G.data_off = dn_words;
        const uint64_t m = G.g1 - G.g0;
        dn_xrows += m;
        dn_words += ((m + 127) / 128) * mg::dense_block_words(G.W);
        sp->dn_wmax = std::max(sp->dn_wmax, G.W);
        for (uint32_t r = G.g0; r < G.g1; r++) grp_of_h[r] = (uint32_t)sp->dgroups_host.size();
        sp->dgroups_host.push_back(G);
    }
    return !sp->dgroups_host.empty();
}

int SparseIndexBuild::encode_groups()
{
    sp->dn_xs = ((s + 7u) & ~7u) + 8u;
    if (!take(&sp->dgroups, sp->dgroups_host.size()) || !take(&sp->grp_of, n) || !take(&sp->gdata, dn_words) || !take(&sp->ext, dn_xrows * sp->dn_xs)) {
        (void)hipGetLastError();
        sp->dgroups_host.clear();
        return MG_OK;
    }
    hipError_t e = hipMemcpyAsync(sp->dgroups, sp->dgroups_host.data(), sp->dgroups_host.size() * sizeof(mg::DenseGroup), hipMemcpyHostToDevice, ctx->stream);
    if (e == hipSuccess) e = hipMemcpyAsync(sp->grp_of, grp_of_h.data(), n * 4, hipMemcpyHostToDevice, ctx->stream);
    if (e == hipSuccess)
        e = mg::launch_dense_encode(sp->off, sp->code_img, sp->pos_img, sp->rs, sp->grp_of, sp->dgroups, sp->ulist, sp->upos, sp->gdata, sp->ext, sp->dn_xs,
                                    (uint32_t)n, sp->dn_wmax, ctx->stream, ctx_opt(ctx, "MASHGPU_DENSE_UL_LDS") ? atoi(ctx_opt(ctx, "MASHGPU_DENSE_UL_LDS")) : -1,
                                    sp->by_tiles ? sp->row_any : nullptr);
    sp->grp_of_host.swap(grp_of_h);
    if (e != hipSuccess) {
        drop();
        drop_dense();
        sp->usable = false;
        return fail(ctx, MG_ERR_HIP, std::string("compare (index build, dense groups): ") + hipGetErrorString(e));
    }
    sp->dn_lists = ctx_opt(ctx, "MASHGPU_DENSE_LISTS") != nullptr;
    return MG_OK;
}

int SparseIndexBuild::dense_groups()
{
    if (!cand_groups.empty()) {
        auto t_dense = std::chrono::steady_clock::now();
        if (built && lead_ready && lead.overflowed() && ctx_opt(ctx, "MASHGPU_SPARSE_DBG"))
            fprintf(stderr, "compare dense: a list of leaders asked for %u entries, room for %u: no dense groups for this table\n", lead.tot[1], lead.cap);
        std::vector<uint32_t> us(cand_groups.size(), 0), ue(cand_groups.size(), 0);
        const int rc = [&] {
            if (!lead_ready || (!built && !search_leaders())) return (int)MG_OK;
            if (lead.tot[0] == 0 || lead.overflowed()) return (int)MG_OK;
            return sort_universes(us, ue) && choose_groups(us, ue) ? encode_groups() : (int)MG_OK;
        }();
        if (rc != MG_OK) return rc;
        if (sp->dgroups_host.empty()) { (void)hipGetLastError(); drop_dense(); }
        sp->build_ms += std::chrono::duration<double, std::milli>(std::chrono::steady_clock::now() - t_dense).count();
        if (ctx_opt(ctx, "MASHGPU_SPARSE_DBG")) {
            uint64_t rows_in = 0;
            for (auto &G : sp->dgroups_host) rows_in += G.g1 - G.g0;
            fprintf(stderr, "compare dense: %zu chains of related rows, %zu groups kept (%llu rows, widest universe %u words)\n", cand_groups.size(),
                    sp->dgroups_host.size(), (unsigned long long)rows_in, sp->dn_wmax);
        }
    }
    if (ctx_opt(ctx, "MASHGPU_SPARSE_DBG")) {
        fprintf(stderr, "compare sparse: index of %llu rows (%llu copies of earlier rows), s %u: %u entries, %u distinct, shared %llu, largest run %u, %.2f ms\n",
                (unsigned long long)n, (unsigned long long)sp->copies, s, E, sp->G, (unsigned long long)sp->shared, sp->max_group, sp->build_ms);
        fprintf(stderr, "compare sparse: rows %s; the copy gate had %u suspects\n",
                !sp->inv ? "in the table's order" : sp->phashes ? "in clustered order, copied" : "in clustered order, read in place", gate_suspects);
    }
    return MG_OK;
}

int SparseIndexBuild::check_row_flags()
{
    if (!ix_verify || !sp->by_tiles || !sp->usable) return MG_OK;
    DevBuf<unsigned long long> d_diff(ctx);
    if (d_diff.alloc(2) != hipSuccess) return no_memory();
    unsigned long long diff[2] = {0, ~0ull};
    hipError_t e = hipMemcpyAsync(d_diff, diff, sizeof diff, hipMemcpyHostToDevice, ctx->stream);
    if (e == hipSuccess) e = mg::index_verify_row_flags(sp->off, sp->code_img, sp->pos_img, sp->rs, sp->row_any, (uint32_t)n, d_diff, ctx->stream);
    if (e == hipSuccess) e = hipMemcpyAsync(diff, d_diff, sizeof diff, hipMemcpyDeviceToHost, ctx->stream);
    if (e == hipSuccess) e = hipStreamSynchronize(ctx->stream);
    if (e != hipSuccess) return lost(e);
    if (diff[0]) {
        sp->usable = false;
        return fail(ctx, MG_ERR_INVALID, "index verify: row flags -- " + std::to_string(diff[0]) + " differ, first at row " + std::to_string(diff[1]));
    }
    return MG_OK;
}

int SparseIndexBuild::run()
{
    int rc = MG_OK;
    if ((rc = scan_rows()) != MG_OK || stop) return rc;
    if ((rc = order_rows()) != MG_OK || stop) return rc;
    if ((rc = find_copies()) != MG_OK || stop) return rc;
    if ((rc = lay_out()) != MG_OK || stop) return rc;
    if ((rc = build_by_tiles()) != MG_OK || stop) return rc;
    if ((rc = build_by_sort()) != MG_OK || stop) return rc;
    if ((rc = check_build()) != MG_OK || stop) return rc;
    if ((rc = dense_groups()) != MG_OK || stop) return rc;
    return check_row_flags();
}

}

int table_sparse_index(mg_ctx *ctx, const mg_table *t, uint32_t s, bool clustered, mg_table::Sparse **out, uint32_t split)
{
    if (!clustered) split = 0;
    for (mg_table::Sparse *sp : t->sparse)
        if (sp->s == s && sp->clustered == clustered && sp->split == split) { *out = sp; return MG_OK; }
    mg_table::Sparse *sp = new mg_table::Sparse;
    sp->s = s;
    sp->clustered = clustered;
    sp->split = split;
    t->sparse.push_back(sp);
    *out = sp;
    auto unusable = [&](const char *why) { sp->usable = false; sp->why = why; return MG_OK; };
    const uint64_t n = t->n;
    if (n == 0) return unusable("empty table");
    if (n >= (1ull << 31)) return unusable("too many rows");
    sp->rs = mg::sparse_img_stride(s);
    if (n * sp->rs >= (1ull << 32)) return unusable("image index beyond 32 bits");
    HIP_TRY(ctx, hipSetDevice(ctx->device));
    SparseIndexBuild build(ctx, t, s, clustered, sp, split);
    prof_begin(ctx, ctx->prof_index);
    struct ProfEnd { mg_ctx *c; ~ProfEnd() { prof_end(c, c->prof_index); } } prof_end_guard{ctx};
    return build.run();
}
```

Baseline: 448.2 billion pairs/s.

## Replace radix sorts in index build with hash tables and per-group LDS sorts

Adds a hash-table path for clustering rows by their first hashes, which replaces the full 64-bit radix sort of n*4 pairs with an atomic-CAS insert and lookup. It also groups universe leaders with a counting scatter into per-group buckets, each bitonic-sorted in LDS, instead of one global radix sort, and a set-based copy gate is declared. The aim is to cut index-build time in every per-step job. Fallbacks to the sort route remain for oversized groups or memory failure, and verify modes compare the new results against the sort.

```diff
diff --git a/mash_amd/csrc/compare_dense.hip b/mash_amd/csrc/compare_dense.hip
--- a/mash_amd/csrc/compare_dense.hip
+++ b/mash_amd/csrc/compare_dense.hip
@@ -182,6 +182,136 @@
 }
 
 #endif
+
+constexpr uint32_t DN_UG_LDS_CAP = 8192;
+constexpr uint32_t DN_UG_BINS = 8192;
+constexpr uint32_t DN_UG_PER = 16, DN_UG_CHUNK = 1024u * DN_UG_PER;
+
+__global__ __launch_bounds__(1024) void dn_ug_count_kernel(const unsigned long long *key, uint32_t m, uint32_t ng, uint32_t *cnt)
+{
+    MG_DYN_SHARED(uint32_t, s_c);
+    const uint32_t t = threadIdx.x, base = blockIdx.x * DN_UG_CHUNK;
+    for (uint32_t b = t; b < ng; b += 1024u) s_c[b] = 0;
+    __syncthreads();
+#pragma unroll
+    for (uint32_t k = 0; k < DN_UG_PER; k++) {
+        const uint32_t i = base + k * 1024u + t;
+        const uint32_t g = i < m ? (uint32_t)(key[i] >> 32) : 0xFFFFFFFFu;
+        if (g < ng) atomicAdd(&s_c[g], 1u);
+    }
+    __syncthreads();
+    for (uint32_t b = t; b < ng; b += 1024u)
+        if (s_c[b]) atomicAdd(&cnt[b], s_c[b]);
+}
+
+__global__ __launch_bounds__(1024) void dn_ug_scan_kernel(uint32_t *cnt, uint32_t ng, uint32_t lds_cap, uint32_t *ustart, uint32_t *uend, uint32_t *flag)
+{
+    __shared__ uint32_t s_w[16];
+    __shared__ uint32_t s_base;
+    const uint32_t t = threadIdx.x, lane = t & 63u, wid = t >> 6;
+    if (t == 0) s_base = 0;
+    __syncthreads();
+    for (uint32_t g0 = 0; g0 < ng; g0 += 1024u) {
+        const uint32_t g = g0 + t;
+        const uint32_t c = g < ng ? cnt[g] : 0u;
+        uint32_t incl = c;
+        for (uint32_t d = 1; d < 64u; d <<= 1) {
+            const uint32_t x = __shfl_up(incl, d);
+            if (lane >= d) incl += x;
+        }
+        if (lane == 63u) s_w[wid] = incl;
+        __syncthreads();
+        uint32_t base = s_base;
+        for (uint32_t k = 0; k < wid; k++) base += s_w[k];
+        if (g < ng) {
+            const uint32_t start = base + incl - c;
+            cnt[g] = start;
+            ustart[g] = c ? start : 0u;
+            uend[g] = c ? start + c : 0u;
+            if (c > lds_cap) atomicMax(flag, 1u);
+        }
+        __syncthreads();
+        if (t == 1023u) s_base = base + incl;
+        __syncthreads();
+    }
+}
+
+__global__ __launch_bounds__(1024) void dn_ug_scatter_kernel(const unsigned long long *key, const uint32_t *val, uint32_t m, uint32_t ng, uint32_t *cursor,
+                                                             unsigned long long *byg)
+{
+    MG_DYN_SHARED(uint32_t, s_c);
+    const uint32_t t = threadIdx.x, base = blockIdx.x * DN_UG_CHUNK;
+    for (uint32_t b = t; b < ng; b += 1024u) s_c[b] = 0;
+    __syncthreads();
+    unsigned long long kk[DN_UG_PER];
+#pragma unroll
+    for (uint32_t k = 0; k < DN_UG_PER; k++) {
+        const uint32_t i = base + k * 1024u + t;
+        kk[k] = i < m ? key[i] : ~0ull;
+        const uint32_t g = (uint32_t)(kk[k] >> 32);
+        if (g < ng) atomicAdd(&s_c[g], 1u);
+    }
+    __syncthreads();
+    for (uint32_t b = t; b < ng; b += 1024u)
+        if (s_c[b]) s_c[b] = atomicAdd(&cursor[b], s_c[b]);
+    __syncthreads();
+#pragma unroll
+    for (uint32_t k = 0; k < DN_UG_PER; k++) {
+        const uint32_t i = base + k * 1024u + t;
+        const uint32_t g = (uint32_t)(kk[k] >> 32);
+        if (g < ng) {
+            const uint32_t at = atomicAdd(&s_c[g], 1u);
+            if (at < m) byg[at] = (kk[k] << 32) | val[i];
+        }
+    }
+}
+
+__global__ __launch_bounds__(512) void dn_ug_sort_kernel(const unsigned long long *byg, const uint32_t *ustart, const uint32_t *uend, uint32_t lds_cap,
+                                                         uint32_t *ulist, uint32_t *upos)
+{
+    MG_DYN_SHARED(unsigned long long, s_e);
+    const uint32_t g = blockIdx.x, tid = threadIdx.x;
+    const uint32_t a = ustart[g], c = uend[g] - a;
+    if (c == 0 || c > lds_cap) return;
+    uint32_t P = 1;
+    while (P < c) P <<= 1;
+    for (uint32_t i = tid; i < P; i += 512u) s_e[i] = i < c ? byg[a + i] : ~0ull;
+    __syncthreads();
+    for (uint32_t k = 2; k <= P; k <<= 1)
+        for (uint32_t j = k >> 1; j > 0; j >>= 1) {
+            for (uint32_t q = tid; q < P / 2u; q += 512u) {
+                const uint32_t i = ((q & ~(j - 1u)) << 1) | (q & (j - 1u)), l = i | j;
+                const unsigned long long x = s_e[i], y = s_e[l];
+                if ((x > y) == ((i & k) == 0)) { s_e[i] = y; s_e[l] = x; }
+            }
+            __syncthreads();
+        }
+    for (uint32_t i = tid; i < c; i += 512u) {
+        ulist[a + i] = (uint32_t)(s_e[i] >> 32);
+        upos[a + i] = (uint32_t)s_e[i];
+    }
+}
+
+uint32_t dense_universe_lds_cap() { return DN_UG_LDS_CAP; }
+bool dense_group_universes_fits(uint32_t ng) { return ng > 0 && ng <= DN_UG_BINS; }
+
+hipError_t dense_group_universes(const unsigned long long *key, const uint32_t *val, uint32_t m, uint32_t ng, uint32_t *cnt, unsigned long long *byg,
+                                 uint32_t *ulist, uint32_t *upos, uint32_t *ustart, uint32_t *uend, uint32_t lds_cap, hipStream_t stream)
+{
+    if (m == 0 || !dense_group_universes_fits(ng) || lds_cap == 0 || (lds_cap & (lds_cap - 1u)) || lds_cap > DN_UG_LDS_CAP) return hipErrorInvalidValue;
+    hipError_t e = hipMemsetAsync(cnt, 0, (((size_t)ng + 1u) * 4u + 15u) & ~(size_t)15u, stream);
+    if (e != hipSuccess) return e;
+    const size_t smem = (size_t)lds_cap * 8u;
+    e = hipFuncSetAttribute(reinterpret_cast<const void *>(dn_ug_sort_kernel), hipFuncAttributeMaxDynamicSharedMemorySize, (int)smem);
+    if (e != hipSuccess) return e;
+    const uint32_t chunks = (m + DN_UG_CHUNK - 1u) / DN_UG_CHUNK;
+    hipLaunchKernelGGL(dn_ug_count_kernel, dim3(chunks), dim3(1024), (size_t)ng * 4u, stream, key, m, ng, cnt);
+    hipLaunchKernelGGL(dn_ug_scan_kernel, dim3(1), dim3(1024), 0, stream, cnt, ng, lds_cap, ustart, uend, cnt + ng);
+    hipLaunchKernelGGL(dn_ug_scatter_kernel, dim3(chunks), dim3(1024), (size_t)ng * 4u, stream, key, val, m, ng, cnt, byg);
+    hipLaunchKernelGGL(dn_ug_sort_kernel, dim3(ng), dim3(512), smem, stream, (const unsigned long long *)byg, (const uint32_t *)ustart, (const uint32_t *)uend,
+                       lds_cap, ulist, upos);
+    return hipGetLastError();
+}
 
 constexpr uint32_t DN_CX_MASK = 0x7FFFu, DN_CX_FLAG = 0x8000u;
 
@@ -639,8 +769,84 @@
     return il >= 8u ? go(dn_pairs_kernel<8, 8>) : go(dn_pairs_kernel<8, 4>);
 }
 
+constexpr uint32_t CL_FIRST = 4;
+
+constexpr unsigned long long CL_EMPTY = ~0ull;
+constexpr uint32_t CL_PROBES = 256;
+
+__device__ __forceinline__ uint32_t cl_slot_of(unsigned long long k, uint32_t mask)
+{
+    k = (k ^ (k >> 33)) * 0xFF51AFD7ED558CCDull;
+    k = (k ^ (k >> 33)) * 0xC4CEB9FE1A85EC53ull;
+    return (uint32_t)(k ^ (k >> 33)) & mask;
+}
+
+__global__ __launch_bounds__(256) void cl_insert_kernel(const uint64_t *hashes, uint64_t stride, const uint32_t *cnt, uint32_t n,
+                                                        unsigned long long *keys, uint32_t *rows, uint32_t mask, uint32_t *full)
+{
+    const uint32_t i = blockIdx.x * 256u + threadIdx.x;
+    if (i >= n * CL_FIRST) return;
+    const uint32_t row = i / CL_FIRST, f = i % CL_FIRST;
+    if (f >= cnt[row]) return;
+    const unsigned long long k = (unsigned long long)hashes[(uint64_t)row * stride + f];
+    if (k == CL_EMPTY) return;
+    uint32_t h = cl_slot_of(k, mask);
+    for (uint32_t probe = 0; probe < CL_PROBES; probe++, h = (h + 1u) & mask) {
+        const unsigned long long was = atomicCAS(&keys[h], CL_EMPTY, k);
+        if (was == CL_EMPTY || was == k) {
+            atomicMin(&rows[h], row);
+            return;
+        }
+    }
+    atomicMin(full, 0u);
+}
+
+__global__ __launch_bounds__(256) void cl_lookup_kernel(const uint64_t *hashes, uint64_t stride, const uint32_t *cnt, uint32_t n,
+                                                        const unsigned long long *keys, const uint32_t *rows, uint32_t mask, uint32_t *label)
+{
+    const uint32_t row = blockIdx.x * 256u + threadIdx.x;
+    if (row >= n) return;
+    const uint32_t c = cnt[row] < CL_FIRST ? cnt[row] : CL_FIRST;
+    uint32_t lab = row;
+    for (uint32_t f = 0; f < c; f++) {
+        const unsigned long long k = (unsigned long long)hashes[(uint64_t)row * stride + f];
+        if (k == CL_EMPTY) continue;
+        uint32_t h = cl_slot_of(k, mask);
+        for (uint32_t probe = 0; probe < CL_PROBES; probe++, h = (h + 1u) & mask) {
+            const unsigned long long at = keys[h];
+            if (at == k) { lab = rows[h] < lab ? rows[h] : lab; break; }
+            if (at == CL_EMPTY) break;
+        }
+    }
+    label[row] = lab;
+}
+
+uint32_t dense_cluster_table_slots(uint32_t n, uint32_t forced)
+{
+    if (forced) return forced;
+    uint32_t slots = 64;
+    while (slots < 8ull * n && slots < (1u << 31)) slots <<= 1;
+    return slots;
+}
+
+size_t dense_cluster_table_bytes(uint32_t slots) { return (size_t)slots * 12u + 16u; }
+
+hipError_t dense_cluster_labels_hash(const uint64_t *hashes, uint64_t stride, const uint32_t *cnt, uint32_t n, void *table, uint32_t slots,
+                                     uint32_t *label, hipStream_t stream, uint32_t *full)
+{
+    if (n == 0 || slots == 0 || (slots & (slots - 1u))) return hipErrorInvalidValue;
+    hipError_t e = hipMemsetAsync(table, 0xFF, dense_cluster_table_bytes(slots), stream);
+    if (e != hipSuccess) return e;
+    unsigned long long *keys = static_cast<unsigned long long *>(table);
+    uint32_t *rows = reinterpret_cast<uint32_t *>(keys + slots);
+    hipLaunchKernelGGL(cl_insert_kernel, dim3((n * CL_FIRST + 255u) / 256u), dim3(256), 0, stream, hashes, stride, cnt, n, keys, rows, slots - 1u,
+                       full ? full : rows + slots);
+    hipLaunchKernelGGL(cl_lookup_kernel, dim3((n + 255u) / 256u), dim3(256), 0, stream, hashes, stride, cnt, n, (const unsigned long long *)keys,
+                       (const uint32_t *)rows, slots - 1u, label);
+    return hipGetLastError();
+}
+
 #ifndef MG_HIP_EMU
-constexpr uint32_t CL_FIRST = 4;
 
 __global__ __launch_bounds__(256) void cl_emit_kernel(const uint64_t *hashes, uint64_t stride, const uint32_t *cnt, uint32_t n,
                                                       unsigned long long *key, uint32_t *row_out, uint32_t *label)
@@ -689,14 +895,38 @@
     }
 }
 
-size_t dense_cluster_temp_bytes(uint32_t n)
+size_t dense_cluster_temp_bytes(uint32_t n, bool pair_sort)
 {
     size_t a = 0, b = 0;
-    rocprim::radix_sort_pairs(nullptr, a, (const unsigned long long *)nullptr, (unsigned long long *)nullptr, (const uint32_t *)nullptr,
-                              (uint32_t *)nullptr, (size_t)n * CL_FIRST, 0u, 64u, (hipStream_t) nullptr);
+    if (pair_sort)
+        rocprim::radix_sort_pairs(nullptr, a, (const unsigned long long *)nullptr, (unsigned long long *)nullptr, (const uint32_t *)nullptr,
+                                  (uint32_t *)nullptr, (size_t)n * CL_FIRST, 0u, 64u, (hipStream_t) nullptr);
     rocprim::radix_sort_keys(nullptr, b, (const unsigned long long *)nullptr, (unsigned long long *)nullptr, (size_t)n, 0u, 64u,
                              (hipStream_t) nullptr);
     return a > b ? a : b;
+}
+
+static hipError_t cl_order_rows(uint32_t n, void *temp, size_t temp_bytes, unsigned long long *key_a, unsigned long long *key_b, uint32_t *lab_a,
+                                uint32_t *lab_b, uint32_t *inv, uint32_t *label_sorted, hipStream_t stream, uint32_t split)
+{
+    hipLaunchKernelGGL(cl_jump_kernel, dim3((n + 255u) / 256u), dim3(256), 0, stream, (const uint32_t *)lab_a, lab_b, n);
+    hipLaunchKernelGGL(cl_jump_kernel, dim3((n + 255u) / 256u), dim3(256), 0, stream, (const uint32_t *)lab_b, lab_a, n);
+    hipLaunchKernelGGL(cl_order_keys_kernel, dim3((n + 255u) / 256u), dim3(256), 0, stream, (const uint32_t *)lab_a, n, split, key_a);
+    hipError_t e = hipGetLastError();
+    if (e != hipSuccess) return e;
+    e = rocprim::radix_sort_keys(temp, temp_bytes, (const unsigned long long *)key_a, key_b, (size_t)n, 0u, 64u, stream);
+    if (e != hipSuccess) return e;
+    hipLaunchKernelGGL(cl_split_keys_kernel, dim3((n + 255u) / 256u), dim3(256), 0, stream, (const unsigned long long *)key_b, n, inv, label_sorted);
+    return hipGetLastError();
+}
+
+hipError_t dense_cluster_rows_hash(const uint64_t *hashes, uint64_t stride, const uint32_t *cnt, uint32_t n, void *temp, size_t temp_bytes, void *table,
+                                   uint32_t slots, unsigned long long *key_a, unsigned long long *key_b, uint32_t *lab_a, uint32_t *lab_b, uint32_t *inv,
+                                   uint32_t *label_sorted, hipStream_t stream, uint32_t split, uint32_t *full)
+{
+    if (n == 0) return hipSuccess;
+    const hipError_t e = dense_cluster_labels_hash(hashes, stride, cnt, n, table, slots, lab_a, stream, full);
+    return e != hipSuccess ? e : cl_order_rows(n, temp, temp_bytes, key_a, key_b, lab_a, lab_b, inv, label_sorted, stream, split);
 }
 
 hipError_t dense_cluster_rows(const uint64_t *hashes, uint64_t stride, const uint32_t *cnt, uint32_t n, void *temp, size_t temp_bytes,
@@ -713,15 +943,7 @@
     if (e != hipSuccess) return e;
     hipLaunchKernelGGL(cl_minrow_kernel, dim3((m + 255u) / 256u), dim3(256), 0, stream, (const unsigned long long *)key_b, (const uint32_t *)row_b, m,
                        lab_a);
-    hipLaunchKernelGGL(cl_jump_kernel, dim3((n + 255u) / 256u), dim3(256), 0, stream, (const uint32_t *)lab_a, lab_b, n);
-    hipLaunchKernelGGL(cl_jump_kernel, dim3((n + 255u) / 256u), dim3(256), 0, stream, (const uint32_t *)lab_b, lab_a, n);
-    hipLaunchKernelGGL(cl_order_keys_kernel, dim3((n + 255u) / 256u), dim3(256), 0, stream, (const uint32_t *)lab_a, n, split, key_a);
-    e = hipGetLastError();
-    if (e != hipSuccess) return e;
-    e = rocprim::radix_sort_keys(temp, temp_bytes, (const unsigned long long *)key_a, key_b, (size_t)n, 0u, 64u, stream);
-    if (e != hipSuccess) return e;
-    hipLaunchKernelGGL(cl_split_keys_kernel, dim3((n + 255u) / 256u), dim3(256), 0, stream, (const unsigned long long *)key_b, n, inv, label_sorted);
-    return hipGetLastError();
+    return cl_order_rows(n, temp, temp_bytes, key_a, key_b, lab_a, lab_b, inv, label_sorted, stream, split);
 }
 
 __global__ __launch_bounds__(256) void cl_gather_rows_kernel(const uint64_t *hashes, uint64_t stride, const uint32_t *inv, uint64_t *out)
diff --git a/mash_amd/csrc/compare_internal.h b/mash_amd/csrc/compare_internal.h
--- a/mash_amd/csrc/compare_internal.h
+++ b/mash_amd/csrc/compare_internal.h
@@ -101,6 +101,17 @@
 hipError_t launch_sparse_dup_suspects(const unsigned long long *dig, const uint32_t *cnt, uint32_t n, void *temp, size_t temp_bytes,
                                       unsigned long long *dig_sorted, uint32_t *rows_sorted, uint32_t *flags, uint32_t *nflag,
                                       hipStream_t stream);
+struct SparseGateTail {
+    uint32_t suspects_less_one, not_full;
+    uint32_t guest, pad;
+    uint32_t suspects() const { return suspects_less_one + 1u; }
+    bool full() const { return not_full != 0xFFFFFFFFu; }
+};
+uint32_t sparse_gate_set_slots(uint32_t n, uint32_t forced = 0);
+size_t sparse_gate_set_bytes(uint32_t slots);
+static inline SparseGateTail *sparse_gate_set_tail(void *set, uint32_t slots) { return reinterpret_cast<SparseGateTail *>(static_cast<unsigned char *>(set) + (size_t)slots * 12u); }
+hipError_t launch_sparse_row_gate_set(const uint64_t *hashes, uint64_t stride, const uint32_t *cnt, uint32_t n, unsigned long long *digest, void *set,
+                                      uint32_t slots, hipStream_t stream);
 size_t sparse_order_temp_bytes(uint32_t n);
 hipError_t launch_sparse_row_order(const uint32_t *off, const uint32_t *code_img, const uint32_t *gend, const uint32_t *rep, uint32_t n,
                                    uint32_t rs, void *temp, size_t temp_bytes, unsigned long long *key_a, unsigned long long *key_b,
@@ -196,6 +207,10 @@
 hipError_t dense_sort_universes(const unsigned long long *key, const uint32_t *val, uint32_t m, void *temp, size_t temp_bytes,
                                 unsigned long long *key_sorted, uint32_t *ulist, uint32_t *upos, uint32_t *ustart, uint32_t *uend,
                                 uint32_t group_bits, hipStream_t stream);
+uint32_t dense_universe_lds_cap();
+bool dense_group_universes_fits(uint32_t ng);
+hipError_t dense_group_universes(const unsigned long long *key, const uint32_t *val, uint32_t m, uint32_t ng, uint32_t *cnt, unsigned long long *byg,
+                                 uint32_t *ulist, uint32_t *upos, uint32_t *ustart, uint32_t *uend, uint32_t lds_cap, hipStream_t stream);
 hipError_t launch_dense_encode(const uint32_t *off, const uint32_t *code_img, uint32_t *pos_img, uint32_t rs, const uint32_t *grp_of,
                                const DenseGroup *groups, const uint32_t *ulist, const uint32_t *upos, unsigned long long *gdata,
                                uint16_t *ext, uint32_t xs, uint32_t n, uint32_t wmax, hipStream_t stream, int ul_mode = -1,
@@ -207,7 +222,14 @@
                               const unsigned long long *gdata, bool use_lists, const uint16_t *ext, uint32_t xs,
                               uint32_t s, uint32_t wmax, uint32_t row_begin, uint32_t row_end, uint64_t out_base, const uint32_t *inv, uint2 *out,
                               hipStream_t stream, const DenseList *list = nullptr);
-size_t dense_cluster_temp_bytes(uint32_t n);
+size_t dense_cluster_temp_bytes(uint32_t n, bool pair_sort = true);
+uint32_t dense_cluster_table_slots(uint32_t n, uint32_t forced = 0);
+size_t dense_cluster_table_bytes(uint32_t slots);
+hipError_t dense_cluster_labels_hash(const uint64_t *hashes, uint64_t stride, const uint32_t *cnt, uint32_t n, void *table, uint32_t slots,
+                                     uint32_t *label, hipStream_t stream, uint32_t *full = nullptr);
+hipError_t dense_cluster_rows_hash(const uint64_t *hashes, uint64_t stride, const uint32_t *cnt, uint32_t n, void *temp, size_t temp_bytes, void *table,
+                                   uint32_t slots, unsigned long long *key_a, unsigned long long *key_b, uint32_t *lab_a, uint32_t *lab_b, uint32_t *inv,
+                                   uint32_t *label_sorted, hipStream_t stream, uint32_t split = 0, uint32_t *full = nullptr);
 hipError_t dense_cluster_rows(const uint64_t *hashes, uint64_t stride, const uint32_t *cnt, uint32_t n, void *temp, size_t temp_bytes,
                               unsigned long long *key_a, unsigned long long *key_b, uint32_t *row_a, uint32_t *row_b, uint32_t *lab_a,
                               uint32_t *lab_b, uint32_t *inv, uint32_t *label_sorted, hipStream_t stream, uint32_t split = 0);
diff --git a/mash_amd/csrc/compare_sparse.hip b/mash_amd/csrc/compare_sparse.hip
--- a/mash_amd/csrc/compare_sparse.hip
+++ b/mash_amd/csrc/compare_sparse.hip
@@ -186,6 +186,75 @@
 {
     const uint64_t stride = (uint64_t)gridDim.x * 256u;
     for (uint64_t i = (uint64_t)blockIdx.x * 256u + threadIdx.x; i < count; i += stride) p[i] = v;
+}
+
+constexpr unsigned long long SP_GATE_EMPTY = ~0ull;
+constexpr uint32_t SP_GATE_PROBES = 256;
+
+__device__ __forceinline__ unsigned long long sp_gate_mix(unsigned long long v, uint32_t p)
+{
+    unsigned long long z = v + 0x9E3779B97F4A7C15ull * (unsigned long long)(p + 1);
+    z = (z ^ (z >> 30)) * 0xBF58476D1CE4E5B9ull;
+    z = (z ^ (z >> 27)) * 0x94D049BB133111EBull;
+    return z ^ (z >> 31);
+}
+
+__device__ __forceinline__ void sp_gate_insert(unsigned long long dig, uint32_t c, unsigned long long *keys, uint32_t *counts, uint32_t mask,
+                                               uint32_t *tail)
+{
+    if (c == 0) return;
+    if (dig == SP_GATE_EMPTY) { atomicAdd(&tail[0], 1u); return; }
+    uint32_t h = (uint32_t)(dig ^ (dig >> 32)) & mask;
+    for (uint32_t probe = 0; probe < SP_GATE_PROBES; probe++, h = (h + 1u) & mask) {
+        const unsigned long long k = atomicCAS(&keys[h], SP_GATE_EMPTY, dig);
+        if (k != SP_GATE_EMPTY && k != dig) continue;
+        const uint32_t cc = atomicCAS(&counts[h], 0xFFFFFFFFu, c);
+        if (cc == 0xFFFFFFFFu) return;
+        if (cc == c) { atomicAdd(&tail[0], 1u); return; }
+    }
+    atomicMin(&tail[1], 0u);
+}
+
+__global__ __launch_bounds__(256) void sp_row_gate_set_kernel(const uint64_t *hashes, uint64_t stride, const uint32_t *cnt, uint32_t nrows,
+                                                              unsigned long long *digest, unsigned long long *keys, uint32_t *counts, uint32_t mask,
+                                                              uint32_t *tail)
+{
+    static_assert(COPY_GATE_SAMPLES == 32, "half a wave per row");
+    const uint32_t row = blockIdx.x * 8u + (threadIdx.x >> 5), k = threadIdx.x & 31u;
+    const uint32_t n = row < nrows ? cnt[row] : 0u;
+    unsigned long long h = 0;
+    if (k < copy_gate_samples(n)) {
+        const uint32_t p = copy_gate_position(k, n);
+        h = sp_gate_mix(hashes[(uint64_t)row * stride + p], p);
+    }
+    for (int d = 16; d > 0; d >>= 1) h += __shfl_xor(h, d);
+    if (k == 0 && row < nrows) {
+        digest[row] = h;
+        sp_gate_insert(h, n, keys, counts, mask, tail);
+    }
+}
+
+uint32_t sparse_gate_set_slots(uint32_t n, uint32_t forced)
+{
+    if (forced) return forced;
+    uint32_t slots = 64;
+    while (slots < 4ull * n && slots < (1u << 31)) slots <<= 1;
+    return slots;
+}
+
+size_t sparse_gate_set_bytes(uint32_t slots) { return (size_t)slots * 12u + 16u; }
+
+hipError_t launch_sparse_row_gate_set(const uint64_t *hashes, uint64_t stride, const uint32_t *cnt, uint32_t n, unsigned long long *digest, void *set,
+                                      uint32_t slots, hipStream_t stream)
+{
+    if (n == 0 || slots == 0 || (slots & (slots - 1u))) return hipErrorInvalidValue;
+    hipError_t e = hipMemsetAsync(set, 0xFF, sparse_gate_set_bytes(slots), stream);
+    if (e != hipSuccess) return e;
+    unsigned long long *keys = static_cast<unsigned long long *>(set);
+    uint32_t *counts = reinterpret_cast<uint32_t *>(keys + slots);
+    hipLaunchKernelGGL(sp_row_gate_set_kernel, dim3((n + 7u) / 8u), dim3(256), 0, stream, hashes, stride, cnt, n, digest, keys, counts, slots - 1u,
+                       counts + slots);
+    return hipGetLastError();
 }
 
 #ifndef MG_HIP_EMU
diff --git a/mash_amd/csrc/host_index.cpp b/mash_amd/csrc/host_index.cpp
--- a/mash_amd/csrc/host_index.cpp
+++ b/mash_amd/csrc/host_index.cpp
@@ -73,11 +73,15 @@
     DevBuf<uint8_t> dc_cls, d_link;
     DevBuf<unsigned long long> dc_last, d_dig, d_dig_sorted, k_a, k_b;
     DevBuf<uint32_t> d_cnt, d_rows_sorted, d_flags, d_nflag, r_a, r_b, l_a, l_b, d_inv, d_lab;
-    DevBuf<unsigned char> d_tmp_dup, d_tmp_cl;
+    DevBuf<unsigned char> d_tmp_dup, d_tmp_cl, d_gate_set, d_cl_tab;
+    bool gate_hash = false, labels_hash = false;
+    uint32_t gate_slots = 0, cl_slots = 0;
+    const char *gate_route = "none", *labels_route = "none", *universes_route = "none";
     std::vector<uint8_t> hc_cls, link;
     std::vector<uint64_t> hc_last;
     std::vector<uint32_t> hc_nh, inv_v, lab_v;
     const uint32_t *inv = nullptr, *lab_sorted = nullptr;
+    uint32_t h_flags[4] = {0, 0, 0, 0};
     uint32_t nflag = 0, gate_suspects = 0;
     size_t tb_dup = 0, tb_cl = 0;
     bool cluster_q = false, links_q = false;
@@ -121,16 +125,38 @@
     std::vector<uint32_t> short_cnt;
 
     bool built = false;
+    int verify_rc = MG_OK;
     uint64_t dn_xrows = 0, dn_words = 0;
 
     SparseIndexBuild(mg_ctx *c, const mg_table *tab, uint32_t sketch_size, bool clustered_variant, mg_table::Sparse *index, uint32_t split_row)
         : ctx(c), t(tab), s(sketch_size), clustered(clustered_variant), split(split_row), sp(index), n(tab->n), dc_cls(c), d_link(c), dc_last(c), d_dig(c), d_dig_sorted(c),
-          k_a(c), k_b(c), d_cnt(c), d_rows_sorted(c), d_flags(c), d_nflag(c), r_a(c), r_b(c), l_a(c), l_b(c), d_inv(c), d_lab(c), d_tmp_dup(c), d_tmp_cl(c), d_lb(c), d_tcnt(c),
+          k_a(c), k_b(c), d_cnt(c), d_rows_sorted(c), d_flags(c), d_nflag(c), r_a(c), r_b(c), l_a(c), l_b(c), d_inv(c), d_lab(c), d_tmp_dup(c), d_tmp_cl(c), d_gate_set(c), d_cl_tab(c), d_lb(c), d_tcnt(c),
           d_groups(c), d_grp_of(c), d_lead_rows(c), lead(c), temp(c), gs_of(c), key64_a(c), key64_b(c), d_stat(c), d_slots(c)
     {}
 
     int unusable(const char *why) { sp->usable = false; sp->why = why; stop = true; return MG_OK; }
 
+    bool opt_is(const char *name, const char *value) const { const char *o = ctx_opt(ctx, name); return o && strcmp(o, value) == 0; }
+    uint32_t opt_pow2(const char *name) const
+    {
+        const char *o = ctx_opt(ctx, name);
+        uint32_t v = o ? (uint32_t)std::min<unsigned long long>(strtoull(o, nullptr, 10), 1u << 30) : 0u, p = v ? 1u : 0u;
+        while (p && 2u * p <= v) p *= 2u;
+        return p;
+    }
+    bool alloc_dup_sort()
+    {
+        if (d_dig_sorted.p && d_rows_sorted.p && d_flags.p && d_nflag.p && d_tmp_dup.p) return true;
+        return d_dig_sorted.alloc(n) == hipSuccess && d_rows_sorted.alloc(n) == hipSuccess && d_flags.alloc(n) == hipSuccess && d_nflag.alloc(1) == hipSuccess &&
+               d_tmp_dup.alloc(std::max<size_t>(tb_dup, 16)) == hipSuccess;
+    }
+    bool alloc_cluster_sort()
+    {
+        tb_cl = mg::dense_cluster_temp_bytes((uint32_t)n);
+        return k_a.alloc(4 * n) == hipSuccess && k_b.alloc(4 * n) == hipSuccess && r_a.alloc(4 * n) == hipSuccess && r_b.alloc(4 * n) == hipSuccess &&
+               l_a.alloc(n) == hipSuccess && l_b.alloc(n) == hipSuccess && d_inv.alloc(n) == hipSuccess && d_lab.alloc(n) == hipSuccess &&
+               d_tmp_cl.alloc(std::max<size_t>(tb_cl, 16)) == hipSuccess;
+    }
 
     bool counts_with_offsets()
     {
@@ -208,6 +234,8 @@
     }
 
     int scan_rows();
+    int verify_scan(const uint32_t *h_inv, const uint32_t *h_lab);
+    int verify_universes(const std::vector<uint32_t> &us, const std::vector<uint32_t> &ue);
     int copy_rows();
     int order_rows();
     int find_copies();
@@ -235,10 +263,14 @@
     try_cluster = clustered && n >= 16;
     try_links = !try_cluster && want_dense && n >= 8 && s <= 16384;
     tb_dup = mg::sparse_dup_temp_bytes((uint32_t)n);
-    tb_cl = mg::dense_cluster_temp_bytes((uint32_t)n);
+    gate_hash = dedup && !opt_is("MASHGPU_COPY_GATE", "sort");
+    labels_hash = try_cluster && !opt_is("MASHGPU_CLUSTER_LABELS", "sort");
+    if (gate_hash) {
+        gate_slots = mg::sparse_gate_set_slots((uint32_t)n, opt_pow2("MASHGPU_COPY_GATE_SLOTS"));
+        if (d_gate_set.alloc(mg::sparse_gate_set_bytes(gate_slots)) != hipSuccess) { (void)hipGetLastError(); gate_hash = false; }
+    }
     if (d_cnt.alloc(n) != hipSuccess || (need_classes && (dc_cls.alloc(n) != hipSuccess || dc_last.alloc(n) != hipSuccess)) ||
-        (dedup && (d_dig.alloc(n) != hipSuccess || d_dig_sorted.alloc(n) != hipSuccess || d_rows_sorted.alloc(n) != hipSuccess ||
-                   d_flags.alloc(n) != hipSuccess || d_nflag.alloc(1) != hipSuccess || d_tmp_dup.alloc(std::max<size_t>(tb_dup, 16)) != hipSuccess))) {
+        (dedup && (d_dig.alloc(n) != hipSuccess || (!gate_hash && !alloc_dup_sort())))) {
         (void)hipGetLastError();
         return unusable("no device memory for the index");
     }
@@ -252,16 +284,34 @@
         }
         if (e == hipSuccess) e = mg::launch_sparse_row_counts(t->nhash, (uint32_t)n, (uint32_t)std::min<uint64_t>(t->s, s), d_cnt, ctx->stream);
         if (e == hipSuccess && dedup) {
-            e = mg::launch_sparse_row_gate(t->hashes, t->s, d_cnt, (uint32_t)n, d_dig, ctx->stream);
-            if (e == hipSuccess)
-                e = mg::launch_sparse_dup_suspects(d_dig, d_cnt, (uint32_t)n, d_tmp_dup, tb_dup, d_dig_sorted, d_rows_sorted, d_flags, d_nflag, ctx->stream);
-        }
-        if (e == hipSuccess && try_cluster) {
-            if (k_a.alloc(4 * n) == hipSuccess && k_b.alloc(4 * n) == hipSuccess && r_a.alloc(4 * n) == hipSuccess && r_b.alloc(4 * n) == hipSuccess &&
-                l_a.alloc(n) == hipSuccess && l_b.alloc(n) == hipSuccess && d_inv.alloc(n) == hipSuccess && d_lab.alloc(n) == hipSuccess &&
-                d_tmp_cl.alloc(std::max<size_t>(tb_cl, 16)) == hipSuccess) {
+            if (gate_hash) {
+                e = mg::launch_sparse_row_gate_set(t->hashes, t->s, d_cnt, (uint32_t)n, d_dig, d_gate_set, gate_slots, ctx->stream);
+            } else {
+                e = mg::launch_sparse_row_gate(t->hashes, t->s, d_cnt, (uint32_t)n, d_dig, ctx->stream);
+                if (e == hipSuccess)
+                    e = mg::launch_sparse_dup_suspects(d_dig, d_cnt, (uint32_t)n, d_tmp_dup, tb_dup, d_dig_sorted, d_rows_sorted, d_flags, d_nflag, ctx->stream);
+            }
+            gate_route = gate_hash ? "hash" : "sort";
+        }
+        if (e == hipSuccess && labels_hash) {
+            cl_slots = mg::dense_cluster_table_slots((uint32_t)n, opt_pow2("MASHGPU_CLUSTER_SLOTS"));
+            tb_cl = mg::dense_cluster_temp_bytes((uint32_t)n, false);
+            if (k_a.alloc(n) == hipSuccess && k_b.alloc(n) == hipSuccess && l_a.alloc(n) == hipSuccess && l_b.alloc(n) == hipSuccess && d_inv.alloc(n) == hipSuccess &&
+                d_lab.alloc(n) == hipSuccess && d_tmp_cl.alloc(std::max<size_t>(tb_cl, 16)) == hipSuccess && d_cl_tab.alloc(mg::dense_cluster_table_bytes(cl_slots)) == hipSuccess) {
+                e = mg::dense_cluster_rows_hash(t->hashes, t->s, d_cnt, (uint32_t)n, d_tmp_cl, tb_cl, d_cl_tab, cl_slots, k_a, k_b, l_a, l_b, d_inv, d_lab, ctx->stream, split,
+                                                gate_hash ? &mg::sparse_gate_set_tail(d_gate_set, gate_slots)->guest : nullptr);
+                cluster_q = true;
+                labels_route = "hash";
+            } else {
+                (void)hipGetLastError();
+                labels_hash = false;
+            }
+        }
+        if (e == hipSuccess && try_cluster && !labels_hash) {
+            if (alloc_cluster_sort()) {
                 e = mg::dense_cluster_rows(t->hashes, t->s, d_cnt, (uint32_t)n, d_tmp_cl, tb_cl, k_a, k_b, r_a, r_b, l_a, l_b, d_inv, d_lab, ctx->stream, split);
                 cluster_q = true;
+                labels_route = "sort";
             } else {
                 (void)hipGetLastError();
             }
@@ -281,14 +331,14 @@
         auto carve = [&](unsigned char *block) {
             Carve c{block};
             p_last = c.take<unsigned long long>(n); p_nh = c.take<uint32_t>(n); p_inv = c.take<uint32_t>(n); p_lab = c.take<uint32_t>(n);
-            p_nflag = c.take<uint32_t>(2); p_cls = c.take<uint8_t>(n); p_link = c.take<uint8_t>(n);
+            p_nflag = c.take<uint32_t>(4); p_cls = c.take<uint8_t>(n); p_link = c.take<uint8_t>(n);
             return c.at + 64;
         };
         unsigned char *pin = static_cast<unsigned char *>(ctx_pinned(ctx, carve(nullptr)));
         if (pin) {
             carve(pin);
         } else {
-            p_nflag = &nflag;
+            p_nflag = h_flags;
             if (cluster_q) { inv_v.resize(n); lab_v.resize(n); p_inv = inv_v.data(); p_lab = lab_v.data(); }
             p_nh = hc_nh.data(); p_cls = hc_cls.data(); p_last = reinterpret_cast<unsigned long long *>(hc_last.data()); p_link = link.data();
         }
@@ -297,7 +347,11 @@
             if (e == hipSuccess) e = hipMemcpyAsync(p_cls, dc_cls, n, hipMemcpyDeviceToHost, ctx->stream);
             if (e == hipSuccess) e = hipMemcpyAsync(p_last, dc_last, n * 8, hipMemcpyDeviceToHost, ctx->stream);
         }
-        if (e == hipSuccess && dedup) e = hipMemcpyAsync(p_nflag, d_nflag, 4, hipMemcpyDeviceToHost, ctx->stream);
+        uint32_t *d_cl_full = labels_hash ? reinterpret_cast<uint32_t *>(d_cl_tab.p + (size_t)cl_slots * 12u) : nullptr;
+        if (e == hipSuccess && dedup)
+            e = gate_hash ? hipMemcpyAsync(p_nflag, mg::sparse_gate_set_tail(d_gate_set, gate_slots), sizeof(mg::SparseGateTail), hipMemcpyDeviceToHost, ctx->stream)
+                          : hipMemcpyAsync(p_nflag, d_nflag, 4, hipMemcpyDeviceToHost, ctx->stream);
+        if (e == hipSuccess && labels_hash && !gate_hash) e = hipMemcpyAsync(p_nflag + 2, d_cl_full, 4, hipMemcpyDeviceToHost, ctx->stream);
         if (e == hipSuccess && cluster_q) {
             e = hipMemcpyAsync(p_inv, d_inv, n * 4, hipMemcpyDeviceToHost, ctx->stream);
             if (e == hipSuccess) e = hipMemcpyAsync(p_lab, d_lab, n * 4, hipMemcpyDeviceToHost, ctx->stream);
@@ -311,11 +365,42 @@
                 memcpy(hc_cls.data(), p_cls, n);
                 memcpy(hc_last.data(), p_last, n * 8);
             }
-            if (dedup) nflag = *p_nflag;
             if (links_q) memcpy(link.data(), p_link, n);
         }
+        if (e == hipSuccess && dedup) nflag = *p_nflag;
+        if (e == hipSuccess && gate_hash) {
+            mg::SparseGateTail tail;
+            memcpy(&tail, p_nflag, sizeof tail);
+            nflag = tail.suspects();
+            if (tail.full()) {
+                gate_route = "sort (the set filled)";
+                gate_hash = false;
+                if (!alloc_dup_sort()) { (void)hipGetLastError(); return unusable("no device memory for the index"); }
+                e = mg::launch_sparse_dup_suspects(d_dig, d_cnt, (uint32_t)n, d_tmp_dup, tb_dup, d_dig_sorted, d_rows_sorted, d_flags, d_nflag, ctx->stream);
+                if (e == hipSuccess) e = hipMemcpyAsync(&nflag, d_nflag, 4, hipMemcpyDeviceToHost, ctx->stream);
+                if (e == hipSuccess) e = hipStreamSynchronize(ctx->stream);
+            }
+        }
+        if (e == hipSuccess && labels_hash && p_nflag[2] != 0xFFFFFFFFu) {
+            labels_route = "sort (the table filled)";
+            cluster_q = labels_hash = false;
+            if (alloc_cluster_sort()) {
+                e = mg::dense_cluster_rows(t->hashes, t->s, d_cnt, (uint32_t)n, d_tmp_cl, tb_cl, k_a, k_b, r_a, r_b, l_a, l_b, d_inv, d_lab, ctx->stream, split);
+                if (e == hipSuccess) e = hipMemcpyAsync(p_inv, d_inv, n * 4, hipMemcpyDeviceToHost, ctx->stream);
+                if (e == hipSuccess) e = hipMemcpyAsync(p_lab, d_lab, n * 4, hipMemcpyDeviceToHost, ctx->stream);
+                const hipError_t ew = hipStreamSynchronize(ctx->stream);
+                if (e == hipSuccess) e = ew;
+                cluster_q = true;
+            } else {
+                (void)hipGetLastError();
+            }
+        }
+        if (e != hipSuccess) return fail(ctx, MG_ERR_HIP, std::string("compare (index: rows, copies, order): ") + hipGetErrorString(e));
+        if (ctx_opt(ctx, "MASHGPU_PREPHASE_VERIFY")) {
+            const int rc = verify_scan(cluster_q ? p_inv : nullptr, cluster_q ? p_lab : nullptr);
+            if (rc != MG_OK) return rc;
+        }
         if (cluster_q) { inv = p_inv; lab_sorted = p_lab; }
-        if (e != hipSuccess) return fail(ctx, MG_ERR_HIP, std::string("compare (index: rows, copies, order): ") + hipGetErrorString(e));
     }
     gate_suspects = nflag;
     if (need_classes) {
@@ -324,6 +409,42 @@
         t->nh.swap(hc_nh);
     }
     if (!links_q) link.clear();
+    return MG_OK;
+}
+
+int SparseIndexBuild::verify_scan(const uint32_t *h_inv, const uint32_t *h_lab)
+{
+    std::string said;
+    if (gate_hash) {
+        uint32_t by_sort = 0;
+        if (!alloc_dup_sort()) return no_memory();
+        HIP_TRY(ctx, mg::launch_sparse_dup_suspects(d_dig, d_cnt, (uint32_t)n, d_tmp_dup, tb_dup, d_dig_sorted, d_rows_sorted, d_flags, d_nflag, ctx->stream));
+        HIP_TRY(ctx, hipMemcpyAsync(&by_sort, d_nflag, 4, hipMemcpyDeviceToHost, ctx->stream));
+        HIP_TRY(ctx, hipStreamSynchronize(ctx->stream));
+        if ((by_sort == 0) != (nflag == 0) || nflag < by_sort)
+            return fail(ctx, MG_ERR_INVALID, "pre-phase verify: copy gate -- " + std::to_string(nflag) + " suspects by the set, " + std::to_string(by_sort) + " by the sort");
+        said += " copy gate " + std::to_string(nflag) + " / " + std::to_string(by_sort) + " suspects;";
+    }
+    if (labels_hash && h_inv && h_lab) {
+        DevBuf<unsigned long long> ka(ctx), kb(ctx);
+        DevBuf<uint32_t> ra(ctx), rb(ctx), la(ctx), lb(ctx), v_inv(ctx), v_lab(ctx);
+        DevBuf<unsigned char> tmp(ctx);
+        const size_t tb = mg::dense_cluster_temp_bytes((uint32_t)n);
+        if (!(ka.alloc(4 * n) == hipSuccess && kb.alloc(4 * n) == hipSuccess && ra.alloc(4 * n) == hipSuccess && rb.alloc(4 * n) == hipSuccess && la.alloc(n) == hipSuccess &&
+              lb.alloc(n) == hipSuccess && v_inv.alloc(n) == hipSuccess && v_lab.alloc(n) == hipSuccess && tmp.alloc(std::max<size_t>(tb, 16)) == hipSuccess))
+            return no_memory();
+        std::vector<uint32_t> s_inv(n), s_lab(n);
+        HIP_TRY(ctx, mg::dense_cluster_rows(t->hashes, t->s, d_cnt, (uint32_t)n, tmp, tb, ka, kb, ra, rb, la, lb, v_inv, v_lab, ctx->stream, split));
+        HIP_TRY(ctx, hipMemcpyAsync(s_inv.data(), v_inv, n * 4, hipMemcpyDeviceToHost, ctx->stream));
+        HIP_TRY(ctx, hipMemcpyAsync(s_lab.data(), v_lab, n * 4, hipMemcpyDeviceToHost, ctx->stream));
+        HIP_TRY(ctx, hipStreamSynchronize(ctx->stream));
+        for (uint64_t a = 0; a < n; a++)
+            if (s_inv[a] != h_inv[a] || s_lab[a] != h_lab[a])
+                return fail(ctx, MG_ERR_INVALID, "pre-phase verify: cluster labels -- index row " + std::to_string(a) + " is row " + std::to_string(h_inv[a]) + " of label " +
+                                                     std::to_string(h_lab[a]) + " by the table, row " + std::to_string(s_inv[a]) + " of label " + std::to_string(s_lab[a]) + " by the sort");
+        said += " cluster labels equal (" + std::to_string(n) + " rows);";
+    }
+    if (ctx_opt(ctx, "MASHGPU_SPARSE_DBG") && !said.empty()) fprintf(stderr, "compare sparse: pre-phase verify:%s\n", said.c_str());
     return MG_OK;
 }
 
@@ -432,6 +553,7 @@
         const int rc = copy_rows();
         if (rc != MG_OK || stop) return rc;
         HIP_TRY(ctx, counts_to_device());
+        if (!alloc_dup_sort()) { (void)hipGetLastError(); return unusable("no device memory for the index"); }
         HIP_TRY(ctx, mg::launch_sparse_row_digest(H, t->s, d_cnt, (uint32_t)n, d_dig, ctx->stream));
         HIP_TRY(ctx, mg::launch_sparse_dup_suspects(d_dig, d_cnt, (uint32_t)n, d_tmp_dup, tb_dup, d_dig_sorted, d_rows_sorted, d_flags, d_nflag, ctx->stream));
         HIP_TRY(ctx, hipMemcpyAsync(&nflag, d_nflag, 4, hipMemcpyDeviceToHost, ctx->stream));
@@ -737,12 +859,39 @@
     const uint32_t ng = (uint32_t)cand_groups.size(), nlead = lead.tot[0];
     uint32_t gbits = 1;
     while ((1u << gbits) < ng) gbits++;
-    const size_t tb = mg::dense_universe_temp_bytes(nlead);
     DevBuf<uint32_t> d_us(ctx), d_ue(ctx);
     DevBuf<unsigned long long> d_key2(ctx);
     DevBuf<unsigned char> d_utmp(ctx);
-    bool ok = d_us.alloc(ng) == hipSuccess && d_ue.alloc(ng) == hipSuccess && d_key2.alloc(nlead) == hipSuccess && d_utmp.alloc(std::max<size_t>(tb, 16)) == hipSuccess;
-    if (!ok || !take(&sp->ulist, nlead) || !take(&sp->upos, nlead)) return false;
+    if (d_key2.alloc(nlead) != hipSuccess ||!take(&sp->ulist, nlead) || !take(&sp->upos, nlead)) return false;
+    if (!opt_is("MASHGPU_DENSE_UNIVERSES", "sort") && !mg::dense_group_universes_fits(ng)) {
+        universes_route = "sort (more groups than counters in LDS)";
+    } else if (!opt_is("MASHGPU_DENSE_UNIVERSES", "sort")) {
+        uint32_t cap = opt_pow2("MASHGPU_DENSE_UNIVERSE_LDS");
+        cap = cap ? std::min(cap, mg::dense_universe_lds_cap()) : mg::dense_universe_lds_cap();
+        DevBuf<uint32_t> d_blk(ctx);
+        if (d_blk.alloc(3ull * ng + 4u) == hipSuccess) {
+            std::vector<uint32_t> back(2ull * ng + 1u);
+            hipError_t e = mg::dense_group_universes(lead.keyj, lead.valj, nlead, ng, d_blk, d_key2, sp->ulist, sp->upos, d_blk + ng + 1u, d_blk + 2ull * ng + 1u, cap, ctx->stream);
+            if (e == hipSuccess) e = hipMemcpyAsync(back.data(), d_blk + ng, back.size() * 4, hipMemcpyDeviceToHost, ctx->stream);
+            const hipError_t ew = hipStreamSynchronize(ctx->stream);
+            if (e != hipSuccess || ew != hipSuccess) return false;
+            if (back[0] == 0) {
+                std::copy(back.begin() + 1, back.begin() + 1 + ng, us.begin());
+                std::copy(back.begin() + 1 + ng, back.end(), ue.begin());
+                universes_route = "groups";
+                if (ctx_opt(ctx, "MASHGPU_PREPHASE_VERIFY")) verify_rc = verify_universes(us, ue);
+                return true;
+            }
+            universes_route = "sort (a group beyond the LDS)";
+        } else {
+            (void)hipGetLastError();
+            universes_route = "sort (no memory)";
+        }
+    } else {
+        universes_route = "sort";
+    }
+    const size_t tb = mg::dense_universe_temp_bytes(nlead);
+    if (!(d_us.alloc(ng) == hipSuccess && d_ue.alloc(ng) == hipSuccess && d_utmp.alloc(std::max<size_t>(tb, 16)) == hipSuccess)) return false;
     hipError_t e = hipMemsetAsync(d_us, 0, ng * 4, ctx->stream);
     if (e == hipSuccess) e = hipMemsetAsync(d_ue, 0, ng * 4, ctx->stream);
     if (e == hipSuccess) e = mg::dense_sort_universes(lead.keyj, lead.valj, nlead, d_utmp, tb, d_key2, sp->ulist, sp->upos, d_us, d_ue, gbits, ctx->stream);
@@ -750,6 +899,37 @@
     if (e == hipSuccess) e = hipMemcpyAsync(ue.data(), d_ue, ng * 4, hipMemcpyDeviceToHost, ctx->stream);
     if (e == hipSuccess) e = hipStreamSynchronize(ctx->stream);
     return e == hipSuccess;
+}
+
+int SparseIndexBuild::verify_universes(const std::vector<uint32_t> &us, const std::vector<uint32_t> &ue)
+{
+    const uint32_t ng = (uint32_t)cand_groups.size(), nlead = lead.tot[0];
+    uint32_t gbits = 1;
+    while ((1u << gbits) < ng) gbits++;
+    const size_t tb = mg::dense_universe_temp_bytes(nlead);
+    DevBuf<uint32_t> d_us(ctx), d_ue(ctx), v_ulist(ctx), v_upos(ctx);
+    DevBuf<unsigned long long> d_key2(ctx);
+    DevBuf<unsigned char> d_utmp(ctx);
+    if (!(d_us.alloc(ng) == hipSuccess && d_ue.alloc(ng) == hipSuccess && v_ulist.alloc(nlead) == hipSuccess && v_upos.alloc(nlead) == hipSuccess &&
+          d_key2.alloc(nlead) == hipSuccess && d_utmp.alloc(std::max<size_t>(tb, 16)) == hipSuccess))
+        return no_memory();
+    std::vector<uint32_t> s_us(ng), s_ue(ng), s_ulist(nlead), s_upos(nlead), g_ulist(nlead), g_upos(nlead);
+    HIP_TRY(ctx, hipMemsetAsync(d_us, 0, ng * 4, ctx->stream));
+    HIP_TRY(ctx, hipMemsetAsync(d_ue, 0, ng * 4, ctx->stream));
+    HIP_TRY(ctx, mg::dense_sort_universes(lead.keyj, lead.valj, nlead, d_utmp, tb, d_key2, v_ulist, v_upos, d_us, d_ue, gbits, ctx->stream));
+    const struct { void *to; const uint32_t *from; size_t words; } copies[6] = {{s_us.data(), d_us, ng}, {s_ue.data(), d_ue, ng}, {s_ulist.data(), v_ulist, nlead},
+                                                                                {s_upos.data(), v_upos, nlead}, {g_ulist.data(), sp->ulist, nlead}, {g_upos.data(), sp->upos, nlead}};
+    for (const auto &c : copies) HIP_TRY(ctx, hipMemcpyAsync(c.to, c.from, c.words * 4, hipMemcpyDeviceToHost, ctx->stream));
+    HIP_TRY(ctx, hipStreamSynchronize(ctx->stream));
+    for (uint32_t g = 0; g < ng; g++)
+        if (us[g] != s_us[g] || ue[g] != s_ue[g])
+            return fail(ctx, MG_ERR_INVALID, "pre-phase verify: universes -- group " + std::to_string(g) + " is [" + std::to_string(us[g]) + ", " + std::to_string(ue[g]) +
+                                                 ") by group, [" + std::to_string(s_us[g]) + ", " + std::to_string(s_ue[g]) + ") by the sort");
+    for (uint32_t i = 0; i < nlead; i++)
+        if (g_ulist[i] != s_ulist[i] || g_upos[i] != s_upos[i])
+            return fail(ctx, MG_ERR_INVALID, "pre-phase verify: universes -- leader " + std::to_string(i) + " differs between the groups' sorts and the sort");
+    if (ctx_opt(ctx, "MASHGPU_SPARSE_DBG")) fprintf(stderr, "compare sparse: pre-phase verify: universes equal (%u leaders in %u groups)\n", nlead, ng);
+    return MG_OK;
 }
 
 bool SparseIndexBuild::choose_groups(const std::vector<uint32_t> &us, const std::vector<uint32_t> &ue)
@@ -812,6 +992,7 @@
             return sort_universes(us, ue) && choose_groups(us, ue) ? encode_groups() : (int)MG_OK;
         }();
         if (rc != MG_OK) return rc;
+        if (verify_rc != MG_OK) return verify_rc;
         if (sp->dgroups_host.empty()) { (void)hipGetLastError(); drop_dense(); }
         sp->build_ms += std::chrono::duration<double, std::milli>(std::chrono::steady_clock::now() - t_dense).count();
         if (ctx_opt(ctx, "MASHGPU_SPARSE_DBG")) {
@@ -824,6 +1005,7 @@
     if (ctx_opt(ctx, "MASHGPU_SPARSE_DBG")) {
         fprintf(stderr, "compare sparse: index of %llu rows (%llu copies of earlier rows), s %u: %u entries, %u distinct, shared %llu, largest run %u, %.2f ms\n",
                 (unsigned long long)n, (unsigned long long)sp->copies, s, E, sp->G, (unsigned long long)sp->shared, sp->max_group, sp->build_ms);
+        fprintf(stderr, "compare sparse: copy gate by %s, cluster labels by %s, universes by %s\n", gate_route, labels_route, universes_route);
         fprintf(stderr, "compare sparse: rows %s; the copy gate had %u suspects\n",
                 !sp->inv ? "in the table's order" : sp->phashes ? "in clustered order, copied" : "in clustered order, read in place", gate_suspects);
     }
```

After: 452.5 billion pairs/s, median of 6. About the same (+0.9%).
